# vdBerg93/cl-rrt

Measured on AMD Instinct MI355X. Metric: nodes expanded/sec (200-obstacle scene), higher is better.
Workload: dtype f64

## Files before the change

### cl-rrt_amd/csrc/clrrt_capi.hip

```cpp
#include <hip/hip_runtime.h>
#include <math.h>

#include <algorithm>
#include <climits>
#include <array>
#include <chrono>
#include <cmath>
#include <cstdio>
#include <cstdlib>
#include <cstring>
#include <deque>
#include <functional>
#include <optional>
#include <string>
#include <vector>

#include "../../include/clrrt.h"
#include "clrrt_dev.hpp"
#include "clrrt_internal.hpp"

static const int kWalkMaxOver = 2048, kWalkMaxChunks = 64;

using namespace clrrt;

// ... 60 lines not shown
  bool nnw_max_over_set = false;
  bool nnw_bud_tiles_set = false;
  int nnw_half_max = 4096;
  int nnw_hscale = 50;
  int nnw_lpt = 0;
  int nnw_index = 5;
  int nnw_lds_floor = 0;
  int nnw_waves = -1;
  int nnw_double = 1;
  WalkBufs nnw{};
  WalkBufs nnw_alt{};
  struct { int64_t n = -1; double ox, oy, x0, y0, x1, y1; float delta; } nnw_built;
  CompactBufs cmp{};
  int roll_persistent = 1;
  int nn_debug = 0;
  int roll_blocks = 0;
  int n_cu = 256;
  int* roll_q = nullptr;
  int* roll_best = nullptr;
  int roll_priority = 1;
  int roll_coop = 1;
  int roll_spread = 1;
  int roll_lanes = 0;
  int nn_exact_fused = 1;
  int exact_min_width = 8;
  int exact_fixup = 1;
  int exact_fix_cap = 0;
  int* fix_n = nullptr;
  int* fix_ids = nullptr;
  int* fix_adj = nullptr;
  NnRec* fix_xrec = nullptr;
  int* fix_xi = nullptr;
  int* fix_xcand = nullptr;
  float* fix_xkey = nullptr;
  int* fix_xn = nullptr;
  std::vector<int> h_fix_cand;
  std::vector<RollRes> h_fix_spec;
  Job* fix_jobs = nullptr;
  RollRes* fix_res = nullptr;
  std::vector<int> h_fix;
  std::vector<clrrt_sample> h_fix_smp;
  std::vector<Job> h_fix_jobs;
  std::vector<int> h_fix_owner;
  std::vector<RollRes> h_fix_res;
  std::vector<SampleOut> h_fix_so;
  int64_t ex_stats[10] = {0, 0, 0, 0, 0, 0, 0, 0, 0, 0};
  int* roll_perm = nullptr;
  int* roll_pflag = nullptr;
  GoalRec* goal_recs = nullptr;
  int* bp_path = nullptr;
  clrrt_node* path_nodes = nullptr;
  double* path_rows = nullptr;
  int path_cap = 0;
  int64_t path_rows_cap = 0;
  int path_n = 0;
  int64_t path_nrows = 0;
  int* ri_int = nullptr;
  int64_t* ri_off = nullptr;
  float* ri_cost = nullptr;
  double* ri_terms = nullptr;
  double reg_x0 = 0, reg_y0 = 0, reg_x1 = 0, reg_y1 = 0;
  int nn_pipeline = 1;
  hipStream_t side = nullptr;
  int cu_split = 0;
  hipStream_t roll_st = nullptr;
  hipEvent_t ev_rs0 = nullptr, ev_rs1 = nullptr;
  hipEvent_t ev_tree = nullptr, ev_walk = nullptr, ev_commit = nullptr;
  clrrt_sample* d_samples2 = nullptr;
  clrrt_sample* h_samples2 = nullptr;
  int* cand2 = nullptr;
  float* ckey2 = nullptr;
  int* ncand2 = nullptr;
  int* ctie2 = nullptr;
  int nn_lag = 0;
  clrrt_sample* d_samples3 = nullptr;
  clrrt_sample* h_samples3 = nullptr;
  int* cand3 = nullptr;
  float* ckey3 = nullptr;
  int* ncand3 = nullptr;
  int* ctie3 = nullptr;
  WalkBufs nnw3{};
  hipStream_t side2 = nullptr;
  hipStream_t mst = nullptr;
  int nn_split_delta = 0;
  int nn_delta_early = 1;
  int nn_lane_order = 1;
  int* nn_order = nullptr;
  float* wseed[3] = {nullptr, nullptr, nullptr};
  hipEvent_t ev_wm[3] = {nullptr, nullptr, nullptr};
  float* nn_seed2 = nullptr;
  float* d1pk[3] = {nullptr, nullptr, nullptr};
  int* d1pi[3] = {nullptr, nullptr, nullptr};
  hipEvent_t ev_d1[3] = {nullptr, nullptr, nullptr};
  hipEvent_t ev_s[3] = {nullptr, nullptr, nullptr};
  hipEvent_t ev_lagw[3] = {nullptr, nullptr, nullptr};
  int stream_prio = 1;
  int walk_cu_reserve = 0;
  hipEvent_t ev_lag[3] = {nullptr, nullptr, nullptr};
  int stream_prio_applied = 0;
  bool side_prio_set = false;
  std::vector<clrrt_sample> pf_next, pf_samples;
  int pf_state = 0;
  struct {
    int T = 0;
    bool active = false;
    int R = 0;
    int T_alloc = 0, n_steps_alloc = 0;
    int64_t vcap = 0;
    RollRes* res = nullptr;
    RollRes* res_gb = nullptr;
    int* cand = nullptr;
    int* ncand = nullptr;
    clrrt_sample* samp = nullptr;
    int* best = nullptr;
    int* dlist[2] = {nullptr, nullptr};
    int cur_dl = 0, nd = 0;
    int nd_eval = -1;
    int* gv = nullptr;
    uint8_t* pend = nullptr;
    void* sel_tmp = nullptr;
    size_t sel_bytes = 0;
    int* d_cnt = nullptr;
    void* carry[2] = {nullptr, nullptr};
    int cur_c = 0, ncarry = 0, carry_cap = 0;
    int64_t round = 0;
    int slot = 0;
    int64_t deferred_total = 0;
  } def;
  struct {
    int rank = 0, world = 1;
    void* dev_local = nullptr;
    int cap_local = 0;
    clrrt_exchange_fn fn = nullptr;
    void* user = nullptr;
    double max_ms = 0;
    int64_t nd_global = 0;
    int64_t rows_stop = 0;
    int last_nb = 0;
    clrrt_node* xbuf = nullptr;
    uint32_t* xkey = nullptr;
    void* xtmp = nullptr;
    size_t xtmp_bytes = 0;
    int64_t xcap = 0;
    unsigned long long* d_goal = nullptr;
    bool poison_seen = false;
    bool fn_failed = false;
  } sh;
  int fail_at_round = 0;
  int fail_after_exchange = 0;
  bool debug_sync = false;
  unsigned long long* dbg_host = nullptr;
  bool iter_log = false;
  std::vector<int64_t> round_sizes;
  std::vector<clrrt_iteration> iters;
  std::vector<SampleOut> iter_tmp;
  clrrt_sample* h_samples = nullptr;
  int64_t* h_totals = nullptr;
  int* h_int = nullptr;
  int64_t last_eval_rows = 0;
  int64_t last_goal_nodes = 0;
  clrrt_counters counters{};
  int64_t nn_bf_keys = 0, nn_samples = 0;
  int64_t nn_super_bounds = 0;
  bool timing = false;
  static constexpr int kKtClasses = 6;
  double kt_ms[kKtClasses] = {};
  int64_t kt_n[kKtClasses] = {};
  std::vector<hipEvent_t> ev_pool;
  std::vector<std::pair<int, std::pair<hipEvent_t, hipEvent_t>>> ev_pending;
};

static void pf_reset(clrrt_ctx* c);
static int flush_replays(clrrt_ctx* c);
static int append_nodes(clrrt_ctx* c, const clrrt_node* dev_nodes, int n);
static int watchdog_check(clrrt_ctx* c);
static void defer_roll_args(clrrt_ctx* c, RollArgs& a, bool capped);
static int commit_round(clrrt_ctx* c, int nn, double elapsed_ms, int* n_app);
// ... 160 lines not shown
  s[31] = 3;
  s[32] = 0;
  s[33] = 0;
  g->pos = 0;
  for (int i = 0; i < 310; i++) clrrt_rng_next(g);
}

int32_t clrrt_rng_next(clrrt_rng* g) {
  int32_t* s = g->r;
  int f = s[31], r = s[32];
  uint32_t v = (uint32_t)s[f] + (uint32_t)s[r];
  s[f] = (int32_t)v;
  int32_t out = (int32_t)(v >> 1);
  f = f + 1 == 31 ? 0 : f + 1;
  r = r + 1 == 31 ? 0 : r + 1;
  s[31] = f;
  s[32] = r;
  return out;
}

int clrrt_draw_samples(const clrrt_params* p, clrrt_rng* rng, int32_t n, clrrt_sample* out) {
  if (!p || !rng || (n > 0 && !out)) return CLRRT_EINVAL;
  const double* g = p->goal;
  const double RM = 2147483647.0;
  double dGoal = sqrt(g[0] * g[0] + g[1] * g[1]);
  double hd = atan2(g[1], g[0]);
  double latMin = -7, latMax = 7;
  float fl = (float)(RM / (dGoal + 10));
  float fw = (float)(RM / (latMax - latMin));
  double ch, sh, cq, sq;
  ::sincos(hd, &sh, &ch);
  ::sincos(hd + M_PI / 2, &sq, &cq);
  for (int j = 0; j < n; j++) {
    double rLong = (float)clrrt_rng_next(rng) / fl;
    double rLat = latMin + (float)clrrt_rng_next(rng) / fw;
    out[j].x = rLong * ch + rLat * cq;
    out[j].y = rLong * sh + rLat * sq;
    double r = (double)clrrt_rng_next(rng) / (double)(2147483647 / 1);
    out[j].explore = r <= ((0 * 0.3) + (1 * 0.7));
    out[j].pad = 0;
  }
  return CLRRT_OK;
}

const char* clrrt_last_error(const clrrt_ctx* c) { return c ? c->err.c_str() : "null context"; }

static void free_all(clrrt_ctx* c) {
  if (c->side) hipStreamSynchronize(c->side);
  void* ptrs[] = {c->tree, c->nn, c->arena, c->obs, c->d_samples, c->pk, c->pi, c->cand, c->ckey, c->ncand,
                  c->ctie, c->sort_scratch, c->res_spec, c->regnodes, c->res_gb, c->gbnodes, c->so, c->first_conflict,
                  c->out_nodes, c->jobs, c->slots, c->rep_buf, c->totals, c->work_ctr, c->grid_buf,
                  c->nn_seed, c->d_bbox, c->roll_q, c->roll_best, c->roll_perm, c->roll_pflag,
                  c->goal_recs, c->bp_path, c->path_nodes, c->path_rows, c->ri_int, c->ri_off, c->ri_cost,
                  c->ri_terms, c->nnw.keys, c->nnw.keys2, c->nnw.vals, c->nnw.vals2, c->nnw.tmp, c->nnw.P, c->nnw.Q,
                  c->nnw.CE, c->nnw.ID, c->nnw.tiles, c->nnw.supers, c->nnw.sorder, c->nnw.HEAD, c->nnw.ovf_n, c->nnw.ovf, c->nnw.pk, c->nnw.pi, c->nnw_alt.keys, c->nnw_alt.keys2, c->nnw_alt.vals, c->nnw_alt.vals2, c->nnw_alt.tmp, c->nnw_alt.P, c->nnw_alt.Q, c->nnw_alt.CE, c->nnw_alt.ID, c->nnw_alt.tiles, c->nnw_alt.supers, c->nnw_alt.sorder, c->nnw_alt.HEAD, c->nnw_alt.ovf_n, c->nnw_alt.ovf, c->nnw_alt.pk, c->nnw_alt.pi, c->nnw.skeys, c->nnw.sids, c->nnw_alt.skeys, c->nnw_alt.sids, c->cmp.packed, c->cmp.scanned,
                  c->cmp.tmp, c->d_samples2, c->cand2, c->ckey2, c->ncand2, c->ctie2, c->d_samples3, c->cand3, c->ckey3,
                  c->ncand3, c->ctie3, c->nnw3.keys, c->nnw3.keys2, c->nnw3.vals, c->nnw3.vals2, c->nnw3.tmp, c->nnw3.P,
                  c->nnw3.Q, c->nnw3.CE, c->nnw3.ID, c->nnw3.tiles, c->nnw3.supers, c->nnw3.sorder, c->nnw3.HEAD,
                  c->nnw3.ovf_n, c->nnw3.ovf, c->nnw3.pk, c->nnw3.pi, c->nnw3.skeys, c->nnw3.sids,
                  c->nnw.trun, c->nnw_alt.trun, c->nnw3.trun, c->nnw.wctr, c->nnw_alt.wctr, c->nnw3.wctr};
  for (void* p : ptrs)
    if (p) hipFree(p);
  void* sptrs[] = {c->sh.xbuf, c->sh.xkey, c->sh.xtmp, c->sh.d_goal, c->fix_n, c->fix_ids, c->fix_jobs, c->fix_res, c->fix_adj,
                   c->fix_xrec, c->fix_xi, c->fix_xcand, c->fix_xkey, c->fix_xn};
  for (void* p : sptrs)
    if (p) hipFree(p);
  void* dptrs[] = {c->def.res, c->def.res_gb, c->def.cand, c->def.ncand, c->def.samp, c->def.best, c->def.dlist[0],
                   c->def.dlist[1], c->def.gv, c->def.pend, c->def.sel_tmp, c->def.d_cnt, c->def.carry[0],
                   c->def.carry[1]};
  for (void* p : dptrs)
    if (p) hipFree(p);
  if (c->h_samples) hipHostFree(c->h_samples);
  if (c->h_samples2) hipHostFree(c->h_samples2);
  if (c->h_samples3) hipHostFree(c->h_samples3);
  if (c->side2) hipStreamSynchronize(c->side2);
  if (c->side2) hipStreamDestroy(c->side2);
  for (auto e : c->ev_lag)
    if (e) hipEventDestroy(e);
  for (auto e : c->ev_lagw)
    if (e) hipEventDestroy(e);
  if (c->mst) hipStreamSynchronize(c->mst);
  if (c->mst) hipStreamDestroy(c->mst);
  for (int q = 0; q < 3; q++) {
    if (c->ev_d1[q]) hipEventDestroy(c->ev_d1[q]);
    if (c->ev_s[q]) hipEventDestroy(c->ev_s[q]);
    if (c->d1pk[q]) hipFree(c->d1pk[q]);
    if (c->wseed[q]) hipFree(c->wseed[q]);
    if (q == 0 && c->nn_order) hipFree(c->nn_order);
    if (c->ev_wm[q]) hipEventDestroy(c->ev_wm[q]);
    if (c->d1pi[q]) hipFree(c->d1pi[q]);
  }
  if (c->nn_seed2) hipFree(c->nn_seed2);
  if (c->side) hipStreamSynchronize(c->side);
  if (c->ev_tree) hipEventDestroy(c->ev_tree);
  if (c->ev_walk) hipEventDestroy(c->ev_walk);
  if (c->ev_commit) hipEventDestroy(c->ev_commit);
  if (c->side) hipStreamDestroy(c->side);
  if (c->roll_st) hipStreamDestroy(c->roll_st);
  if (c->ev_rs0) hipEventDestroy(c->ev_rs0);
  if (c->ev_rs1) hipEventDestroy(c->ev_rs1);
  if (c->h_totals) hipHostFree(c->h_totals);
  if (c->h_int) hipHostFree(c->h_int);
  if (c->h_bbox) hipHostFree(c->h_bbox);
  if (c->dbg_host) hipHostFree(c->dbg_host);
  for (auto& pe : c->ev_pending) { hipEventDestroy(pe.second.first); hipEventDestroy(pe.second.second); }
  for (auto e : c->ev_pool) hipEventDestroy(e);
  if (c->own_stream && c->stream) hipStreamDestroy(c->stream);
}

int clrrt_create(const clrrt_params* p, const clrrt_capacity* cap, int device, clrrt_ctx** out) {
  if (!p || !out) return CLRRT_EINVAL;
  *out = nullptr;
  int ndev = 0;
  if (hipGetDeviceCount(&ndev) != hipSuccess || ndev <= 0) return CLRRT_EHIP;
  if (device < 0 || device >= ndev) return CLRRT_EINVAL;
  clrrt_ctx* c = new clrrt_ctx();
  c->device = device;
  c->params = *p;
  c->debug_sync = getenv("CLRRT_DEBUG_SYNC") != nullptr;
  clrrt_capacity dc;
  dc.max_nodes = 1 << 20;
  dc.max_rows = 1 << 24;
  dc.max_batch = 4096;
  dc.max_obstacles = 4096;
  c->cap = cap ? *cap : dc;
  if (c->cap.max_nodes < 2 || c->cap.max_rows < 2 || c->cap.max_batch < 1 || c->cap.max_obstacles < 0) {
    delete c;
    return CLRRT_EINVAL;
  }
  derive(c->params, c->dp, 0);
  int rc = CLRRT_OK;
  auto chk = [&](hipError_t e) {
    if (e != hipSuccess && rc == CLRRT_OK) { rc = CLRRT_EHIP; c->err = hipGetErrorString(e); }
  };
  chk(hipSetDevice(device));
  chk(hipStreamCreateWithFlags(&c->stream, hipStreamNonBlocking));
  c->own_stream = true;
  const int64_t B = c->cap.max_batch;
  chk(dalloc(&c->tree, c->cap.max_nodes));
  chk(dalloc(&c->nn, c->cap.max_nodes));
  chk(dalloc(&c->arena, (size_t)c->cap.max_rows * 10));
  chk(dalloc(&c->obs, std::max<int64_t>(1, c->cap.max_obstacles)));
  chk(dalloc(&c->d_samples, B));
  c->partial_cap = std::max<int64_t>(B * 16, 4096) * NN_K;
  chk(dalloc(&c->pk, c->partial_cap));
  chk(dalloc(&c->pi, c->partial_cap));
  chk(dalloc(&c->cand, B * CAND_K));
  chk(dalloc(&c->ckey, B * CAND_K));
  chk(dalloc(&c->ncand, B));
  chk(dalloc(&c->ctie, B));
  chk(dalloc(&c->d_samples2, B));
  chk(dalloc(&c->cand2, B * CAND_K));
  chk(dalloc(&c->ckey2, B * CAND_K));
  chk(dalloc(&c->ncand2, B));
  chk(dalloc(&c->ctie2, B));
  chk(hipStreamCreateWithFlags(&c->side, hipStreamNonBlocking));
  chk(hipEventCreateWithFlags(&c->ev_tree, hipEventDisableTiming));
  chk(hipEventCreateWithFlags(&c->ev_walk, hipEventDisableTiming));
  chk(hipEventCreateWithFlags(&c->ev_commit, hipEventDisableTiming));
  chk(dalloc(&c->res_spec, B * CAND_K));
  chk(dalloc(&c->regnodes, B));
  chk(dalloc(&c->res_gb, B * CAND_K));
  c->slot_rows = 0;
  chk(hipMalloc(&c->rep_buf, replay_bytes() * (size_t)2 * B));
  chk(dalloc(&c->gbnodes, B));
  chk(dalloc(&c->so, B));
  chk(dalloc(&c->first_conflict, 1));
  chk(dalloc(&c->out_nodes, 2 * B));
  chk(dalloc(&c->jobs, 2 * B));
  chk(dalloc(&c->totals, 8));
  chk(dalloc(&c->cmp.packed, B));
  chk(dalloc(&c->cmp.scanned, B));
  c->cmp.tmp_bytes = compact_scan_bytes((int)B);
  chk(hipMalloc(&c->cmp.tmp, std::max<size_t>(c->cmp.tmp_bytes, 256)));
  chk(dalloc(&c->nn_seed, B));
// ... 602 lines not shown

int clrrt_work_counters(clrrt_ctx* c, int64_t out[3]) {
  if (!c || !out) return CLRRT_EINVAL;
  HIPC(c, hipSetDevice(c->device));
  unsigned long long h[4];
  HIPC(c, hipMemcpyAsync(h, c->work_ctr, sizeof(h), hipMemcpyDeviceToHost, c->stream));
  HIPC(c, hipStreamSynchronize(c->stream));
  for (int i = 0; i < 3; i++) out[i] = (int64_t)h[i];
  return CLRRT_OK;
}

int clrrt_search_work(clrrt_ctx* c, int64_t out[4]) {
  if (!c || !out) return CLRRT_EINVAL;
  HIPC(c, hipSetDevice(c->device));
  HIPC(c, hipStreamSynchronize(c->stream));
  if (c->side) HIPC(c, hipStreamSynchronize(c->side));
  unsigned long long h[19];
  HIPC(c, hipMemcpy(h, c->work_ctr + 8, sizeof(h), hipMemcpyDeviceToHost));
  out[0] = c->nn_bf_keys;
  out[1] = c->nn_samples;
  out[2] = (int64_t)h[11];
  out[3] = (int64_t)h[13];
  return CLRRT_OK;
}

int clrrt_search_work_ex(clrrt_ctx* c, int64_t out[8]) {
  if (!c || !out) return CLRRT_EINVAL;
  int64_t w[4];
  const int rc = clrrt_search_work(c, w);
  if (rc != CLRRT_OK) return rc;
  unsigned long long h[19];
  HIPC(c, hipMemcpy(h, c->work_ctr + 8, sizeof(h), hipMemcpyDeviceToHost));
  for (int i = 0; i < 4; i++) out[i] = w[i];
  out[4] = c->nn_super_bounds;
  out[5] = (int64_t)h[10];
  out[6] = (int64_t)h[12];
  out[7] = 0;
  return CLRRT_OK;
}

int clrrt_nn_stats(clrrt_ctx* c, int64_t out[19]) {
  if (!c || !out) return CLRRT_EINVAL;
  HIPC(c, hipSetDevice(c->device));
  HIPC(c, hipStreamSynchronize(c->stream));
  unsigned long long h[19];
  HIPC(c, hipMemcpy(h, c->work_ctr + 8, sizeof(h), hipMemcpyDeviceToHost));
  for (int i = 0; i < 19; i++) out[i] = (int64_t)h[i];
  out[4] &= 0xffffffff;
  return CLRRT_OK;
}

int clrrt_set_option(clrrt_ctx* c, const char* key, int64_t value) {
  if (!c || !key) return CLRRT_EINVAL;
  const std::string k(key);
  if (k == "roll_persistent") c->roll_persistent = value != 0;
  else if (k == "nn_walk_min" && value >= 0) c->nnw_min_nodes = value;
  else if (k == "nn_walk_stateless") c->nnw_stateless = value != 0;
  else if (k == "nn_walk_budget_tiles" && value >= 0 && value < INT_MAX) {
    c->nnw_bud_tiles = (int)value;
    c->nnw_bud_tiles_set = true;
  }
  else if (k == "nn_walk_budget_keys" && value >= 0 && value < INT_MAX) c->nnw_bud_ex = (int)value;
  else if (k == "nn_walk_half_max" && value >= 0 && value < INT_MAX) c->nnw_half_max = (int)value;
  else if (k == "nn_walk_hscale" && value >= 1 && value <= 10000) {
    c->nnw_hscale = (int)value;
    c->nnw_built.n = -1;
    c->nnw.sorted_n = c->nnw_alt.sorted_n = c->nnw3.sorted_n = -1;
  }
  else if (k == "nn_walk_lpt") c->nnw_lpt = value != 0;
  else if (k == "nn_walk_index" && value >= 0 && value <= 5) {
    c->nnw_index = (int)value;
    c->nnw_built.n = -1;
    c->nnw.sorted_n = c->nnw_alt.sorted_n = c->nnw3.sorted_n = -1;
  }
  else if (k == "nn_walk_lds_floor" && value >= 0 && value <= 65536) c->nnw_lds_floor = (int)value;
  else if (k == "nn_walk_waves" && value >= -1 && value <= 1 << 20) c->nnw_waves = (int)value;
  else if (k == "nn_walk_chunks" && value >= 1 && value <= kWalkMaxChunks) c->nnw_chunks = (int)value;
  else if (k == "nn_walk_max_over" && value >= 1 && value <= kWalkMaxOver) {
    c->nnw_max_over = (int)value;
    c->nnw_max_over_set = true;
  }
  else if (k == "nn_walk_double") c->nnw_double = value != 0;
  else if (k == "nn_lag" && (value == 0 || value == 1 || value == 2)) c->nn_lag = (int)value;
  else if (k == "nn_split_delta") c->nn_split_delta = value != 0 ? 1 : 0;
  else if (k == "nn_delta_early") c->nn_delta_early = value != 0 ? 1 : 0;
  else if (k == "nn_lane_order") c->nn_lane_order = value != 0 ? 1 : 0;
  else if (k == "nn_debug" && value >= 0) c->nn_debug = (int)value;
  else if (k == "fail_at_round" && value >= 0 && value < INT_MAX) c->fail_at_round = (int)value;
  else if (k == "fail_after_exchange" && value >= 0 && value < INT_MAX) c->fail_after_exchange = (int)value;
  else if (k == "roll_blocks" && value >= 0 && value < (1 << 20)) c->roll_blocks = (int)value;
  else if (k == "nn_pipeline") c->nn_pipeline = value != 0;
  else if (k == "roll_priority") c->roll_priority = value != 0;
  else if (k == "roll_coop") c->roll_coop = value != 0;
  else if (k == "roll_spread") c->roll_spread = value != 0;
  else if (k == "roll_lanes") c->roll_lanes = (int)std::max<int64_t>(0, std::min<int64_t>(64, value));
  else if (k == "nn_exact_fused") c->nn_exact_fused = value != 0;
  else if (k == "rows_deferred") {
    int rc = flush_replays(c);
    if (rc != CLRRT_OK) return rc;
    c->rows_deferred = value != 0;
  }
  else if (k == "exact_min_width" && value >= 1 && value <= 1 << 20) c->exact_min_width = (int)value;
  else if (k == "exact_fixup") c->exact_fixup = value != 0;
  else if (k == "exact_fixup_cap" && value >= 0 && value < INT_MAX) c->exact_fix_cap = (int)value;
  else if (k == "defer_steps" && value >= 0 && value <= 1 << 20) {
    if (value > 0 && value < 8) return fail(c, CLRRT_EINVAL, "defer_steps must be 0 or >= 8");
    c->def.T = (int)value;
  }
  else if (k == "cu_split" && value >= 0 && value <= 7) {
    HIPC(c, hipStreamSynchronize(c->side));
    if (c->roll_st) HIPC(c, hipStreamSynchronize(c->roll_st));
    HIPC(c, hipStreamDestroy(c->side));
    c->side = nullptr;
    if (c->roll_st) HIPC(c, hipStreamDestroy(c->roll_st));
    c->roll_st = nullptr;
    c->cu_split = (int)value;
    c->stream_prio_applied = 0;
    if (value == 0) {
      HIPC(c, hipStreamCreateWithFlags(&c->side, hipStreamNonBlocking));
    } else {
      const int nw = (c->n_cu + 31) / 32;
      std::vector<uint32_t> mr(nw, 0u), ms(nw, 0u);
      for (int i = 0; i < c->n_cu; i++) ((i % 8) < value ? mr : ms)[i / 32] |= 1u << (i % 32);
      HIPC(c, hipExtStreamCreateWithCUMask(&c->roll_st, (uint32_t)nw, mr.data()));
      HIPC(c, hipExtStreamCreateWithCUMask(&c->side, (uint32_t)nw, ms.data()));
      if (!c->ev_rs0) HIPC(c, hipEventCreateWithFlags(&c->ev_rs0, hipEventDisableTiming));
      if (!c->ev_rs1) HIPC(c, hipEventCreateWithFlags(&c->ev_rs1, hipEventDisableTiming));
    }
  }
  else if (k == "stream_prio") c->stream_prio = value != 0;
  else if (k == "walk_cu_reserve" && value >= 0 && value <= 7) c->walk_cu_reserve = (int)value;
  else if (k == "side_priority") {
    int lo = 0, hi = 0;
    HIPC(c, hipDeviceGetStreamPriorityRange(&lo, &hi));
    HIPC(c, hipStreamSynchronize(c->side));
    HIPC(c, hipStreamDestroy(c->side));
    const int pr = value > 0 ? hi : value < 0 ? lo : 0;
    HIPC(c, hipStreamCreateWithPriority(&c->side, hipStreamNonBlocking, pr));
    c->side_prio_set = true;
    c->stream_prio_applied = 0;
    if (value < 0 && c->own_stream) {
      HIPC(c, hipStreamSynchronize(c->stream));
      HIPC(c, hipStreamDestroy(c->stream));
      HIPC(c, hipStreamCreateWithPriority(&c->stream, hipStreamNonBlocking, hi));
    }
  }
  else return fail(c, CLRRT_EINVAL, "unknown option or value: " + k);
  return CLRRT_OK;
}

int clrrt_enable_timing(clrrt_ctx* c, int32_t on) {
  if (!c) return CLRRT_EINVAL;
  drain_timers(c);
  c->timing = on != 0;
  for (int i = 0; i < clrrt_ctx::kKtClasses; i++) { c->kt_ms[i] = 0; c->kt_n[i] = 0; }
  return CLRRT_OK;
}

int clrrt_kernel_time(clrrt_ctx* c, int32_t which, double* ms, int64_t* launches) {
  if (!c || which < 0 || which >= clrrt_ctx::kKtClasses) return CLRRT_EINVAL;
  drain_timers(c);
  if (ms) *ms = c->kt_ms[which];
  if (launches) *launches = c->kt_n[which];
  return CLRRT_OK;
}

}
// ... 996 lines not shown
  c->sh.poison_seen = c->sh.fn_failed = false;
}

static int commit_round(clrrt_ctx* c, int nn, double elapsed_ms, int* n_app) {
  auto& h = c->sh;
  *n_app = 0;
  if (h.world <= 1) {
    *n_app = nn;
    const int rc = append_nodes(c, c->out_nodes, nn);
    if (rc == CLRRT_OK) c->round_sizes.push_back(c->n_nodes);
    return rc;
  }
  if (nn > h.cap_local) return fail(c, CLRRT_ECAPACITY, "the round's records exceed the exchange buffer");
  std::optional<KTimer> kt;
  kt.emplace(c, 5);
  if (nn > 0)
    HIPC(c, hipMemcpyAsync(h.dev_local, c->out_nodes, sizeof(clrrt_node) * nn, hipMemcpyDeviceToDevice, c->stream));
  clrrt_exchange_io io;
  memset(&io, 0, sizeof(io));
  io.n_local = nn;
  io.elapsed_ms = elapsed_ms;
  const int64_t nd_loc = c->def.active ? c->def.nd : 0;
  const bool rows_full =
      c->n_rows + nn + 2 * ((int64_t)h.last_nb + nd_loc) * (c->dp.n_steps_max + 1) > c->cap.max_rows;
  io.aux_local = nd_loc + (rows_full ? (1ll << 32) : 0);
  for (int q = 0; q < 4; q++) io.bbox_local[q] = nn > 0 ? c->h_bbox[q] : (q < 2 ? HUGE_VAL : -HUGE_VAL);
  io.stream = (void*)c->stream;
  io.max_elapsed_ms = elapsed_ms;
  io.aux_sum = io.aux_local;
  if (h.fn(h.user, &io) != 0 || io.n_all < 0 || (io.n_all > 0 && !io.dev_all)) {
    h.fn_failed = true;
    return fail(c, CLRRT_EHIP, "the exchange of the round's records failed");
  }
  kt.reset();
  const int64_t aux_sum = io.aux_sum;
  if (aux_sum >> 48) {
    h.poison_seen = true;
    return fail(c, CLRRT_EHIP, "sharded expansion: " + std::to_string(aux_sum >> 48) + " rank(s) failed this round");
  }
  if (c->fail_after_exchange > 0 && --c->fail_after_exchange == 0)
    return fail(c, CLRRT_ECAPACITY, "injected failure (option fail_after_exchange)");
  h.max_ms = io.max_elapsed_ms;
  h.nd_global = aux_sum & 0xffffffffll;
  h.rows_stop = (aux_sum >> 32) & 0xffff;
  const int32_t n_all = io.n_all;
  void* all = io.dev_all;
  if (n_all > 0) {
    if (n_all > h.xcap) {
      HIPC(c, hipStreamSynchronize(c->stream));
      for (void* p : {(void*)h.xbuf, (void*)h.xkey, h.xtmp})
        if (p) HIPC(c, hipFree(p));
      h.xbuf = nullptr; h.xkey = nullptr; h.xtmp = nullptr;
      const int64_t cap = std::max<int64_t>(2 * (int64_t)n_all, 4096);
      HIPC(c, dalloc(&h.xbuf, cap));
      HIPC(c, dalloc(&h.xkey, 4 * cap));
      h.xtmp_bytes = xorder_sort_bytes((int)cap);
      HIPC(c, hipMalloc(&h.xtmp, std::max<size_t>(h.xtmp_bytes, 256)));
      h.xcap = cap;
    }
    HIPC(c, launch_xorder(c->stream, (const clrrt_node*)all, n_all, c->def.active, h.xkey, h.xtmp, h.xtmp_bytes,
                          h.xbuf, h.d_goal));
    int rc = append_nodes(c, h.xbuf, n_all);
    if (rc != CLRRT_OK) return rc;
    bbox_add(c, io.bbox_all[0], io.bbox_all[1], io.bbox_all[2], io.bbox_all[3]);
  }
  *n_app = n_all;
  c->round_sizes.push_back(c->n_nodes);
  return CLRRT_OK;
}

struct LagSlot {
  clrrt_sample* d = nullptr;
  clrrt_sample* h = nullptr;
  int* cand = nullptr;
  float* ckey = nullptr;
  int* ncand = nullptr;
  int* ctie = nullptr;
  hipEvent_t ev = nullptr;
  hipEvent_t evw = nullptr;
  int n = 0;
  int64_t g = 0;
  int64_t tree_n = 0;
  int stream = 0;
  float* d1pk = nullptr;
  int* d1pi = nullptr;
  int d1_chunks = 0;
  int64_t d1_count = 0;
  hipEvent_t evd1 = nullptr;
  hipEvent_t evs = nullptr;
  float* wseed = nullptr;
  hipEvent_t evm = nullptr;
};

static int lag_alloc(clrrt_ctx* c) {
  if (c->side2) return CLRRT_OK;
  const int64_t B = c->cap.max_batch;
  HIPC(c, dalloc(&c->d_samples3, B));
  HIPC(c, dalloc(&c->cand3, B * CAND_K));
  HIPC(c, dalloc(&c->ckey3, B * CAND_K));
  HIPC(c, dalloc(&c->ncand3, B));
  HIPC(c, dalloc(&c->ctie3, B));
  HIPC(c, hipHostMalloc((void**)&c->h_samples3, sizeof(clrrt_sample) * B, hipHostMallocDefault));
  for (auto& e : c->ev_lag) HIPC(c, hipEventCreateWithFlags(&e, hipEventDisableTiming));
  for (auto& e : c->ev_lagw) HIPC(c, hipEventCreateWithFlags(&e, hipEventDisableTiming));
  if (c->cu_split > 0) {
    const int nw = (c->n_cu + 31) / 32;
    std::vector<uint32_t> ms(nw, 0u);
    for (int i = 0; i < c->n_cu; i++)
      if ((i % 8) >= c->cu_split) ms[i / 32] |= 1u << (i % 32);
    HIPC(c, hipExtStreamCreateWithCUMask(&c->side2, (uint32_t)nw, ms.data()));
  } else {
    HIPC(c, hipStreamCreateWithFlags(&c->side2, hipStreamNonBlocking));
  }
  HIPC(c, hipStreamCreateWithFlags(&c->mst, hipStreamNonBlocking));
  HIPC(c, dalloc(&c->nn_seed2, B));
  for (int q = 0; q < 3; q++) {
    HIPC(c, dalloc(&c->d1pk[q], c->partial_cap));
    HIPC(c, dalloc(&c->wseed[q], B));
    if (q == 0) HIPC(c, dalloc(&c->nn_order, B));
    HIPC(c, hipEventCreateWithFlags(&c->ev_wm[q], hipEventDisableTiming));
    HIPC(c, dalloc(&c->d1pi[q], c->partial_cap));
    HIPC(c, hipEventCreateWithFlags(&c->ev_d1[q], hipEventDisableTiming));
    HIPC(c, hipEventCreateWithFlags(&c->ev_s[q], hipEventDisableTiming));
  }
  return CLRRT_OK;
}

static int apply_stream_prio(clrrt_ctx* c) {
  const int want = (c->stream_prio ? 1 : 2) + 4 * c->walk_cu_reserve;
  if (c->stream_prio_applied == want || c->cu_split > 0) return CLRRT_OK;
  int lo = 0, hi = 0;
  HIPC(c, hipDeviceGetStreamPriorityRange(&lo, &hi));
  const int p_hi = c->stream_prio ? hi : 0, p_lo = c->stream_prio ? lo : 0;
  HIPC(c, hipDeviceSynchronize());
  auto remake = [&](hipStream_t& st, int pr) -> int {
    if (st) HIPC(c, hipStreamDestroy(st));
    HIPC(c, hipStreamCreateWithPriority(&st, hipStreamNonBlocking, pr));
    return CLRRT_OK;
  };
  int rc;
  if (c->walk_cu_reserve > 0) {
    const int nw = (c->n_cu + 31) / 32;
    std::vector<uint32_t> ms(nw, 0u);
    for (int i = 0; i < c->n_cu; i++)
      if ((i % 8) >= c->walk_cu_reserve) ms[i / 32] |= 1u << (i % 32);
    for (hipStream_t* st : {&c->side, &c->side2}) {
      if (*st) HIPC(c, hipStreamDestroy(*st));
      HIPC(c, hipExtStreamCreateWithCUMask(st, (uint32_t)nw, ms.data()));
    }
    if ((rc = remake(c->mst, p_hi)) != CLRRT_OK) return rc;
  } else if ((!c->side_prio_set && (rc = remake(c->side, p_lo)) != CLRRT_OK) ||
             (rc = remake(c->side2, p_lo)) != CLRRT_OK || (rc = remake(c->mst, p_hi)) != CLRRT_OK) {
    return rc;
  }
  if (c->own_stream && (rc = remake(c->stream, p_hi)) != CLRRT_OK) return rc;
  c->stream_prio_applied = want;
  return CLRRT_OK;
}

static int expand_lag2(clrrt_ctx* c, clrrt_rng* rng, int64_t n_iters, double budget_ms, int32_t batch,
                       clrrt_stats* out) {
  int rc = lag_alloc(c);
  if (rc == CLRRT_OK) rc = apply_stream_prio(c);
  if (rc == CLRRT_OK) rc = defer_begin(c, true);
  if (rc != CLRRT_OK) return rc;
  clrrt_stats st{};
  const auto t0 = std::chrono::steady_clock::now();
  clrrt_rng work = *rng, committed = *rng;
  std::deque<clrrt_sample> pending;
  const int cur = batch;
  const bool sharded = c->sh.world > 1;
  c->sh.max_ms = 0;
  c->sh.nd_global = 0;
  c->sh.rows_stop = 0;
  shard_expansion_begin(c);
  if (sharded && (rc = shard_goal_reset(c)) != CLRRT_OK) return rc;
  const int64_t nodes_before = c->n_nodes;
  hipStream_t sides[2] = {c->side, c->side2};
  WalkBufs* W[3] = {&c->nnw, &c->nnw_alt, &c->nnw3};
  int64_t built_n[3] = {-1, -1, -1};
  double built_f[3][7] = {};
  LagSlot A, B;
  A.d = c->d_samples2; A.h = c->h_samples2; A.cand = c->cand2; A.ckey = c->ckey2; A.ncand = c->ncand2;
  A.ctie = c->ctie2; A.ev = c->ev_lag[0]; A.evw = c->ev_lagw[0];
  B.d = c->d_samples3; B.h = c->h_samples3; B.cand = c->cand3; B.ckey = c->ckey3; B.ncand = c->ncand3;
  B.ctie = c->ctie3; B.ev = c->ev_lag[1]; B.evw = c->ev_lagw[1];
  A.d1pk = c->d1pk[0]; A.d1pi = c->d1pi[0]; A.evd1 = c->ev_d1[0]; A.evs = c->ev_s[0];
  B.d1pk = c->d1pk[1]; B.d1pi = c->d1pi[1]; B.evd1 = c->ev_d1[1]; B.evs = c->ev_s[1];
  A.wseed = c->wseed[0]; A.evm = c->ev_wm[0];
  B.wseed = c->wseed[1]; B.evm = c->ev_wm[1];
  float* cur_wseed = c->wseed[2];
  hipEvent_t cur_evm = c->ev_wm[2];
  const bool early = c->nn_delta_early != 0;
  hipEvent_t cur_ev = c->ev_lag[2];
  hipEvent_t cur_evw = c->ev_lagw[2];
  float* cur_d1pk = c->d1pk[2];
  int* cur_d1pi = c->d1pi[2];
  hipEvent_t cur_evd1 = c->ev_d1[2], cur_evs = c->ev_s[2];
  const bool split_delta = c->nn_split_delta != 0;
  struct RoleGuard {
    std::function<void()> f;
    ~RoleGuard() { f(); }
  } role_guard{[&]() {
    c->d_samples2 = A.d; c->h_samples2 = A.h; c->cand2 = A.cand; c->ckey2 = A.ckey; c->ncand2 = A.ncand; c->ctie2 = A.ctie;
    c->d_samples3 = B.d; c->h_samples3 = B.h; c->cand3 = B.cand; c->ckey3 = B.ckey; c->ncand3 = B.ncand; c->ctie3 = B.ctie;
    c->ev_lag[0] = A.ev; c->ev_lag[1] = B.ev; c->ev_lag[2] = cur_ev;
    c->ev_lagw[0] = A.evw; c->ev_lagw[1] = B.evw; c->ev_lagw[2] = cur_evw;
    c->nnw_built.n = -1;
    c->nnw.sorted_n = -1;
    c->nnw_alt.sorted_n = -1;
    c->nnw3.sorted_n = -1;
  }};
  bool have_cur = false;
  int cur_stream = 0;
  double last_round_ms = 0;
  auto frame_of = [](const NnSetup& su, double* f) {
    f[0] = su.fr.ox; f[1] = su.fr.oy; f[2] = su.fr.delta; f[3] = su.x0; f[4] = su.y0; f[5] = su.x1; f[6] = su.y1;
  };
  auto build = [&](int k, const NnSetup& su) -> int {
    double f[7];
    frame_of(su, f);
    if (built_n[k] == c->n_nodes && std::equal(f, f + 7, built_f[k])) return CLRRT_OK;
    int r2 = ensure_walk_set(c, *W[k]);
    if (r2 != CLRRT_OK) return r2;
    const WalkBufs* prev = nullptr;
    for (int q = 1; q <= 2 && !prev; q++) {
      const WalkBufs* w = W[(k + 3 - q) % 3];
      if (w->P && w->sorted_n > 0) prev = w;
    }
    KTimer kt(c, 0, c->stream);
    HIPC(c, launch_nn_walk_build(c->stream, c->nn, (int)c->n_nodes, su.fr, su.x0, su.y0, su.x1, su.y1, *W[k], prev));
    built_n[k] = c->n_nodes;
    std::copy(f, f + 7, built_f[k]);
    return CLRRT_OK;
  };
  auto walk = [&](LagSlot& sl, int n, int k, const NnSetup& su, int si) -> int {
    hipStream_t s = sides[si];
    int r2 = ensure_walk_set(c, *W[k]);
    if (r2 != CLRRT_OK) return r2;
    c->nn_bf_keys += (int64_t)n * c->n_nodes;
    c->nn_samples += n;
    HIPC(c, hipStreamWaitEvent(s, c->ev_tree, 0));
    HIPC(c, hipMemcpyAsync(sl.d, sl.h, sizeof(clrrt_sample) * n, hipMemcpyHostToDevice, s));
    HIPC(c, hipEventRecord(sl.evs, s));
    sl.d1_count = 0;
    sl.d1_chunks = 0;
    c->nn_super_bounds += (int64_t)n * walk_super_count(c->n_nodes);
    {
      KTimer kt(c, 0, s), kt3(c, 3, s);
      W[k]->seed_out = early ? sl.wseed : nullptr;
      W[k]->ev_main = early ? sl.evm : nullptr;
      const hipError_t ew = launch_nn_walk_search(s, sl.d, n, c->nn, (int)c->n_nodes, c->dp, su.fr, su.x0, su.y0, su.x1,
                                                  su.y1, *W[k], sl.cand, sl.ckey, sl.ncand, sl.ctie, c->work_ctr + 18,
                                                  c->nnw_stateless);
      W[k]->seed_out = nullptr;
      W[k]->ev_main = nullptr;
      HIPC(c, ew);
    }
    HIPC(c, hipEventRecord(sl.evw, s));
    sl.n = n;
    sl.tree_n = c->n_nodes;
    sl.stream = si;
    return CLRRT_OK;
  };
  auto draw_to = [&](int64_t want) {
    while ((int64_t)pending.size() < want) {
      clrrt_sample smp;
      clrrt_draw_samples(&c->params, &work, 1, &smp);
      pending.push_back(smp);
    }
  };
  for (int64_t k = 0; rc == CLRRT_OK; k++) {
    const auto tr0 = std::chrono::steady_clock::now();
    if (n_iters > 0 && st.iterations >= n_iters) break;
    const double ms0 = std::chrono::duration<double, std::milli>(tr0 - t0).count();
    if (n_iters == 0 && !((sharded ? c->sh.max_ms : ms0) < budget_ms)) break;
    const int64_t left = n_iters > 0 ? n_iters - st.iterations : INT64_MAX;
    const int64_t gb = std::min<int64_t>(cur, left);
    int64_t f0 = 0;
    int nb = (int)gb;
    if (sharded) shard_slice(c, gb, &f0, &nb);
    c->sh.last_nb = nb;
    const int64_t nc = gb + (sharded ? c->sh.nd_global : (int64_t)c->def.nd);
    if (c->n_nodes + 2 * nc > c->cap.max_nodes ||
        (sharded ? c->sh.rows_stop > 0 : c->n_rows + 2 * nc * (c->dp.n_steps_max + 1) > c->cap.max_rows)) {
      if (n_iters > 0) { rc = fail(c, CLRRT_ECAPACITY, "tree capacity exhausted"); break; }
      st.capacity_stop = 1;
      break;
    }
    const int wk = (int)(k % 3);
    const NnSetup su = nn_setup(c);
    const bool serve = c->n_nodes >= c->nnw_min_nodes && su.region_ok;
    int64_t gA = 0, gB = 0, fA = 0, fB = 0;
    int nA = 0, nB = 0;
    if (serve) {
      const bool more = n_iters > 0 || ms0 + 2.0 * last_round_ms < budget_ms;
      if (A.n == 0 && (n_iters > 0 || ms0 + last_round_ms < budget_ms)) gA = std::max<int64_t>(0, std::min<int64_t>(cur, left - gb));
      const int64_t gA_eff = A.n > 0 ? A.g : gA;
      if (more && gA_eff > 0) gB = std::max<int64_t>(0, std::min<int64_t>(cur, left - gb - gA_eff));
      nA = (int)gA;
      nB = (int)gB;
      if (sharded) {
        shard_slice(c, gA, &fA, &nA);
        shard_slice(c, gB, &fB, &nB);
      }
    }
    const int64_t gA_all = A.n > 0 ? A.g : gA;
    draw_to(gb + gA_all + gB);
    if (have_cur) {
      KTimer kt(c, 4);
      HIPC(c, hipStreamWaitEvent(c->stream, cur_ev, 0));
    } else {
      for (int j = 0; j < nb; j++) c->h_samples[j] = pending[f0 + j];
      HIPC(c, hipMemcpyAsync(c->d_samples, c->h_samples, sizeof(clrrt_sample) * nb, hipMemcpyHostToDevice, c->stream));
      if (serve) {
        HIPC(c, hipStreamSynchronize(c->side));
        HIPC(c, hipStreamSynchronize(c->side2));
        HIPC(c, hipStreamSynchronize(c->mst));
        if ((rc = build(wk, su)) != CLRRT_OK) break;
        c->nn_bf_keys += (int64_t)nb * c->n_nodes;
        c->nn_samples += nb;
        c->nn_super_bounds += (int64_t)nb * walk_super_count(c->n_nodes);
        KTimer kt(c, 0), kt3(c, 3);
        HIPC(c, launch_nn_walk_search(c->stream, c->d_samples, nb, c->nn, (int)c->n_nodes, c->dp, su.fr, su.x0, su.y0,
                                      su.x1, su.y1, *W[wk], c->cand, c->ckey, c->ncand, c->ctie, c->work_ctr + 18,
                                      c->nnw_stateless));
      } else if ((rc = run_nn(c, nb, nullptr)) != CLRRT_OK) {
        break;
      }
    }
    if (serve && (nA > 0 || nB > 0) && (rc = build(wk, su)) != CLRRT_OK) break;
    auto ahead = [&]() -> int {
      if (nA > 0) {
        for (int j = 0; j < nA; j++) A.h[j] = pending[gb + fA + j];
        const int r2 = walk(A, nA, wk, su, cur_stream);
        if (r2 != CLRRT_OK) return r2;
        A.g = gA;
      }
      if (nB > 0) {
        for (int j = 0; j < nB; j++) B.h[j] = pending[gb + gA_all + fB + j];
        const int r2 = walk(B, nB, wk, su, nA > 0 ? A.stream : 1 - A.stream);
        if (r2 != CLRRT_OK) return r2;
        B.g = gB;
      }
      return CLRRT_OK;
    };
    int L = nb, nn = 0, n_app = 0;
    if ((rc = eval_samples(c, nb, false, &L, true, (nA > 0 || nB > 0) ? std::function<int()>(ahead) : nullptr,
                           nullptr)) != CLRRT_OK)
      break;
    if ((rc = compact_and_copy(c, L, &nn, true)) != CLRRT_OK) break;
    const double ms_commit = std::chrono::duration<double, std::milli>(std::chrono::steady_clock::now() - t0).count();
    if ((rc = commit_round(c, nn, ms_commit, &n_app)) != CLRRT_OK) break;
    if ((A.n > 0 || (split_delta && B.n > 0)))
      HIPC(c, hipEventRecord(c->ev_commit, c->stream));
    if (A.n > 0 && split_delta) {
      hipStream_t s = c->mst;
      HIPC(c, hipStreamWaitEvent(s, c->ev_commit, 0));
      HIPC(c, hipStreamWaitEvent(s, early ? A.evm : A.evw, 0));
      const int64_t first2 = A.tree_n + A.d1_count, cnt2 = c->n_nodes - first2;
      int nch2 = 0;
      if (cnt2 > 0) {
        KTimer kt(c, 0, s);
        c->nn_bf_keys += (int64_t)A.n * cnt2;
        const NnSetup su2 = nn_setup(c);
        const int max_chunks = (int)std::max<int64_t>(1, c->partial_cap / ((int64_t)A.n * NN_K));
        HIPC(c, launch_nn_delta_partial(s, A.d, A.n, c->nn, (int)first2, (int)cnt2, c->dp, su2.fr, c->pk, c->pi,
                                        max_chunks, A.ckey, A.ncand, early ? A.wseed : c->nn_seed, early,
                                        c->nn_lane_order ? c->nn_order : nullptr, &nch2));
      }
      if (early) HIPC(c, hipStreamWaitEvent(s, A.evw, 0));
      if (A.d1_count > 0) HIPC(c, hipStreamWaitEvent(s, A.evd1, 0));
      {
        KTimer kt(c, 0, s);
        if (A.d1_count > 0)
          HIPC(c, launch_nn_delta_merge(s, A.n, A.d1_chunks, c->dp, A.d1pk, A.d1pi, (int)A.tree_n, A.cand, A.ckey,
                                        A.ncand, A.ctie));
        HIPC(c, launch_nn_delta_merge(s, A.n, nch2, c->dp, c->pk, c->pi, (int)first2, A.cand, A.ckey, A.ncand, A.ctie));
      }
      HIPC(c, hipEventRecord(A.ev, s));
    } else if (A.n > 0 && early) {
      hipStream_t s = c->mst;
      HIPC(c, hipStreamWaitEvent(s, c->ev_commit, 0));
      HIPC(c, hipStreamWaitEvent(s, A.evm, 0));
      const int64_t first = A.tree_n, cnt = c->n_nodes - A.tree_n;
      int nch = 0;
      if (cnt > 0) {
        KTimer kt(c, 0, s);
        c->nn_bf_keys += (int64_t)A.n * cnt;
        const NnSetup su2 = nn_setup(c);
        const int max_chunks = (int)std::max<int64_t>(1, c->partial_cap / ((int64_t)A.n * NN_K));
        HIPC(c, launch_nn_delta_partial(s, A.d, A.n, c->nn, (int)first, (int)cnt, c->dp, su2.fr, c->pk, c->pi,
                                        max_chunks, nullptr, nullptr, A.wseed, true,
                                        c->nn_lane_order ? c->nn_order : nullptr, &nch));
      }
      HIPC(c, hipStreamWaitEvent(s, A.evw, 0));
      {
        KTimer kt(c, 0, s);
        HIPC(c, launch_nn_delta_merge(s, A.n, nch, c->dp, c->pk, c->pi, (int)first, A.cand, A.ckey, A.ncand, A.ctie));
      }
      HIPC(c, hipEventRecord(A.ev, s));
    } else if (A.n > 0) {
      hipStream_t s = c->mst;
      HIPC(c, hipStreamWaitEvent(s, c->ev_commit, 0));
      HIPC(c, hipStreamWaitEvent(s, A.evw, 0));
      const int64_t first = A.tree_n, cnt = c->n_nodes - A.tree_n;
      if (cnt > 0) {
        KTimer kt(c, 0, s);
        c->nn_bf_keys += (int64_t)A.n * cnt;
        const NnSetup su2 = nn_setup(c);
        const int max_chunks = (int)std::max<int64_t>(1, c->partial_cap / ((int64_t)A.n * NN_K));
        HIPC(c, launch_nn_delta(s, A.d, A.n, c->nn, (int)first, (int)cnt, c->dp, su2.fr, c->pk, c->pi, max_chunks,
                                A.cand, A.ckey, A.ncand, A.ctie, c->nn_seed));
      }
      HIPC(c, hipEventRecord(A.ev, s));
    }
    if (split_delta && B.n > 0) {
      hipStream_t s2 = c->mst;
      HIPC(c, hipStreamWaitEvent(s2, c->ev_commit, 0));
      HIPC(c, hipStreamWaitEvent(s2, B.evs, 0));
      HIPC(c, hipStreamWaitEvent(s2, early ? B.evm : B.evw, 0));
      const int64_t cnt1 = c->n_nodes - B.tree_n;
      B.d1_count = cnt1;
      B.d1_chunks = 0;
      if (cnt1 > 0) {
        KTimer kt(c, 0, s2);
        c->nn_bf_keys += (int64_t)B.n * cnt1;
        const NnSetup su1 = nn_setup(c);
        const int max_chunks = (int)std::max<int64_t>(1, c->partial_cap / ((int64_t)B.n * NN_K));
        HIPC(c, launch_nn_delta_partial(s2, B.d, B.n, c->nn, (int)B.tree_n, (int)cnt1, c->dp, su1.fr, B.d1pk, B.d1pi,
                                        max_chunks, B.ckey, B.ncand, early ? B.wseed : c->nn_seed2, early,
                                        c->nn_lane_order ? c->nn_order : nullptr, &B.d1_chunks));
      }
      HIPC(c, hipEventRecord(B.evd1, s2));
    }
    {
      const NnSetup sn = nn_setup(c);
      if (B.n > 0 && c->n_nodes >= c->nnw_min_nodes && sn.region_ok && (rc = build((int)((k + 1) % 3), sn)) != CLRRT_OK)
        break;
    }
    for (int64_t j = 0; j < gb; j++) {
      pending.pop_front();
      for (int q = 0; q < 3; q++) clrrt_rng_next(&committed);
    }
    st.iterations += gb;
    st.goal_nodes_added += c->last_goal_nodes;
    st.speculated += gb;
    st.rounds++;
    {
      LagSlot old;
      old.d = c->d_samples; old.h = c->h_samples; old.cand = c->cand; old.ckey = c->ckey; old.ncand = c->ncand;
      old.ctie = c->ctie; old.ev = cur_ev; old.evw = cur_evw; old.stream = cur_stream;
      old.d1pk = cur_d1pk; old.d1pi = cur_d1pi; old.evd1 = cur_evd1; old.evs = cur_evs;
      old.wseed = cur_wseed; old.evm = cur_evm;
      have_cur = A.n > 0;
      c->d_samples = A.d; c->h_samples = A.h; c->cand = A.cand; c->ckey = A.ckey; c->ncand = A.ncand; c->ctie = A.ctie;
      cur_ev = A.ev;
      cur_evw = A.evw;
      cur_stream = A.stream;
      cur_d1pk = A.d1pk; cur_d1pi = A.d1pi; cur_evd1 = A.evd1; cur_evs = A.evs;
      cur_wseed = A.wseed; cur_evm = A.evm;
      A = B;
      B = old;
      B.n = 0;
      B.stream = 1 - A.stream;
    }
    last_round_ms = std::chrono::duration<double, std::milli>(std::chrono::steady_clock::now() - tr0).count();
  }
  if (rc == CLRRT_OK) rc = defer_drain(c, &st.goal_nodes_added);
  st.deferred = c->def.deferred_total;
  if (rc == CLRRT_OK) rc = flush_replays(c);
  if (rc == CLRRT_OK && sharded) rc = shard_goal_count(c, &st.goal_nodes_added);
  rc = shard_expansion_end(c, rc);
  c->def.active = false;
  for (hipStream_t s : {c->side, c->side2, c->mst, c->stream}) {
    const hipError_t e = hipStreamSynchronize(s);
    if (e != hipSuccess && rc == CLRRT_OK) rc = fail(c, CLRRT_EHIP, std::string("hipStreamSynchronize: ") + hipGetErrorString(e));
  }
  st.nodes_added = c->n_nodes - nodes_before;
  st.elapsed_ms = std::chrono::duration<double, std::milli>(std::chrono::steady_clock::now() - t0).count();
  *rng = committed;
  if (out) *out = st;
  return rc;
}

int clrrt_expand(clrrt_ctx* c, clrrt_rng* rng, int64_t n_iters, double budget_ms, int32_t mode, int32_t batch,
                 clrrt_stats* out) {
  if (!c || !rng || n_iters < 0 || (mode != CLRRT_MODE_EXACT && mode != CLRRT_MODE_BATCH)) return CLRRT_EINVAL;
  pf_reset(c);
  if (n_iters == 0 && !(budget_ms > 0)) return CLRRT_EINVAL;
  if (c->n_nodes <= 0) return fail(c, CLRRT_ESTATE, "tree not initialised");
  c->round_sizes.clear();
  const bool sharded = c->sh.world > 1;
  if (sharded && mode != CLRRT_MODE_BATCH) return fail(c, CLRRT_EINVAL, "sharded expansion runs BATCH rounds only");
  HIPC(c, hipSetDevice(c->device));
  const int64_t bmax = (int64_t)c->cap.max_batch * c->sh.world;
  batch = (int32_t)std::max<int64_t>(1, std::min<int64_t>(batch > 0 ? batch : bmax, bmax));
  if (sharded && batch < c->sh.world) return fail(c, CLRRT_EINVAL, "fewer samples per round than ranks");
  const int lag = c->nn_lag ? c->nn_lag
                  : (n_iters == 0 ? budget_ms >= 1000.0 : n_iters >= 64 * (int64_t)batch) ? 2 : 1;
  if (mode == CLRRT_MODE_BATCH && c->nn_pipeline && lag == 2) return expand_lag2(c, rng, n_iters, budget_ms, batch, out);
  clrrt_stats st{};
  auto t0 = std::chrono::steady_clock::now();
  clrrt_rng work = *rng;
  clrrt_rng committed = *rng;
  std::deque<clrrt_sample> pending;
  const bool exact = mode == CLRRT_MODE_EXACT;
  int cur = exact ? std::min(batch, std::max(16, c->exact_min_width)) : batch;
  int64_t nodes_before = c->n_nodes;
  int rc = defer_begin(c, !exact);
  c->sh.max_ms = 0;
  c->sh.nd_global = 0;
  c->sh.rows_stop = 0;
  shard_expansion_begin(c);
  if (rc == CLRRT_OK && sharded) rc = shard_goal_reset(c);
  bool have_next = false;
  double last_round_ms = 0;
  auto draw_to = [&](int64_t want) {
    while ((int64_t)pending.size() < want) {
      clrrt_sample smp;
      clrrt_draw_samples(&c->params, &work, 1, &smp);
      pending.push_back(smp);
    }
  };
  for (; rc == CLRRT_OK;) {
    const auto tr0 = std::chrono::steady_clock::now();
    if (n_iters > 0 && st.iterations >= n_iters) break;
    if (n_iters == 0) {
      double ms = std::chrono::duration<double, std::milli>(std::chrono::steady_clock::now() - t0).count();
      if (!((sharded ? c->sh.max_ms : ms) < budget_ms)) break;
    }
    int64_t gb = cur;
    if (n_iters > 0) gb = std::min<int64_t>(gb, n_iters - st.iterations);
    int64_t f0 = 0;
    int nb = (int)gb;
    if (sharded) shard_slice(c, gb, &f0, &nb);
    c->sh.last_nb = nb;
    const int64_t nc = gb + (sharded ? c->sh.nd_global : (int64_t)c->def.nd);
    if (c->n_nodes + 2 * nc > c->cap.max_nodes ||
        (sharded ? c->sh.rows_stop > 0 : c->n_rows + 2 * nc * (c->dp.n_steps_max + 1) > c->cap.max_rows)) {
      if (n_iters > 0) { rc = fail(c, CLRRT_ECAPACITY, "tree capacity exhausted"); break; }
      st.capacity_stop = 1;
      break;
// ... 357 lines not shown
```

### cl-rrt_amd/csrc/clrrt_internal.hpp

```cpp
#pragma once
#include <hip/hip_runtime.h>
#include <stdint.h>

#include "../../include/clrrt.h"
#include "clrrt_dev.hpp"
#include "clrrt_stdsort.hpp"

namespace clrrt {

#define CLRRT_ROLL_PENDING (-2)

struct RollRes {
  double st[10];
  double costE, costS;
  double bx, by;
  double fx, fy;
  double vback;
  int32_t outcome;
  int32_t nrows;
  int32_t refN;
  int32_t pad;
};

struct WorkCtr {
// ... 87 lines not shown
  const float* __restrict__ ckey;
  const int* __restrict__ ncand;
  const RollRes* __restrict__ res;
  const RollRes* __restrict__ res_gb;
  clrrt_node* regnodes;
  clrrt_node* gbnodes;
  SampleOut* so;
  int B;
  const int* view;
  int nd, sbase;
  int* gv;
  uint8_t* pend;
  int* new_pend;
};

struct NnFrame {
  double ox, oy;
  float delta;
  int debug;
};
struct WalkTile {
  float pcx, pcy, pr;
  float rcx, rcy, rr;
  float thx, thy, thh;
  float apx, apy, aph;
  float cemin;
  float aopt;
  int32_t nonfinite;
  float eroot;
};
static_assert(sizeof(WalkTile) == 64, "WalkTile layout");
struct WalkBufs {
  uint32_t *keys, *keys2;
  int *vals, *vals2;
  int* sorder;
  void* tmp;
  size_t tmp_bytes;
  float4 *P, *Q;
  float* CE;
  int* ID;
  int* HEAD;
  int2* trun;
  WalkTile *tiles, *supers;
  int bud_tiles, bud_ex, max_over, nch;
  int half_max = 4096;
  int lds_floor = 0;
  int waves = 0;
  int waves_min_batch = 0;
  int index_kind = 0;
  int hscale_pct = 100;
  int* wctr = nullptr;
  int lpt = 0;
  float* seed_out = nullptr;
  hipEvent_t ev_main = nullptr;
  int* ovf_n;
  int4* ovf;
  float* pk;
  int* pi;
  uint64_t* skeys;
  int* sids;
  int64_t sorted_n;
  double sorted_x0, sorted_y0, sorted_scale;
  int sorted_kind;
  int64_t cap_nodes;
  int cap_batch;
};
size_t walk_sort_bytes(int n);
int64_t walk_tile_count(int64_t n);
int64_t walk_super_count(int64_t n);
hipError_t launch_nn_walk(hipStream_t st, const clrrt_sample* S, int B, const NnRec* nodes, int N, const DevParams& p,
                          const NnFrame& fr, double x0, double y0, double x1, double y1, WalkBufs& w, int* cand,
                          float* ckey, int* ncand, int* ctie, unsigned long long* stats, bool stateless);
hipError_t launch_nn_walk_build(hipStream_t st, const NnRec* nodes, int N, const NnFrame& fr, double x0, double y0,
                                double x1, double y1, WalkBufs& w, const WalkBufs* prev = nullptr);
hipError_t launch_nn_walk_search(hipStream_t st, const clrrt_sample* S, int B, const NnRec* nodes, int N,
                                 const DevParams& p, const NnFrame& fr, double x0, double y0, double x1, double y1,
                                 WalkBufs& w, int* cand, float* ckey, int* ncand, int* ctie, unsigned long long* stats,
                                 bool stateless);
hipError_t launch_walk_audit(hipStream_t st, const clrrt_sample* S, int B, const NnRec* nodes, int N, const DevParams& p,
                             const NnFrame& fr, const WalkBufs& w, int* out);
hipError_t launch_nn_delta(hipStream_t st, const clrrt_sample* S, int B, const NnRec* nodes, int first, int count,
                           const DevParams& p, const NnFrame& fr, float* pk, int* pi, int max_chunks, int* cand,
                           float* ckey, int* ncand, int* ctie, float* seed);
hipError_t launch_nn_delta_partial(hipStream_t st, const clrrt_sample* S, int B, const NnRec* nodes, int first,
                                   int count, const DevParams& p, const NnFrame& fr, float* pk, int* pi, int max_chunks,
                                   const float* ckey, const int* ncand, float* gcap, bool seeded, int* order,
                                   int* nchunks_out);
hipError_t launch_nn_delta_merge(hipStream_t st, int B, int nchunks, const DevParams& p, const float* pk, const int* pi,
                                 int id0, int* cand, float* ckey, int* ncand, int* ctie);
hipError_t launch_nn(hipStream_t st, const clrrt_sample* S, int B, const NnRec* nodes, int N,
                     const DevParams& p, float* pk, int* pi, int* cand, float* ckey, int* ncand, int* ctie,
                     int max_chunks, KeyId* exact_scratch, float* seed, unsigned long long* stats, const NnFrame& fr);
hipError_t launch_nn_exact_only(hipStream_t st, const clrrt_sample* S, int B, const NnRec* nodes, int N,
                                const DevParams& p, const int* ctie, KeyId* scratch, int* cand, float* ckey,
                                int* ncand);
hipError_t launch_rollout(hipStream_t st, int src, const RollArgs& a);
hipError_t launch_nn_exact_small(hipStream_t st, const clrrt_sample* S, int B, const NnRec* nodes, int N,
                                 const DevParams& p, int* cand, float* ckey, int* ncand, int* ctie);
int nn_exact_small_max();
hipError_t launch_rollout_persistent(hipStream_t st, const RollArgs& a, int B, int* qnext, int* best, int blocks,
                                     bool prefilled = false);
struct FillInts {
  int* p[8];
  int n[8];
  int v[8];
  int nj = 0;
  void add(int* ptr, int count, int value) {
    if (ptr && count > 0) { p[nj] = ptr; n[nj] = count; v[nj] = value; nj++; }
  }
};
hipError_t launch_fill_ints(hipStream_t st, const FillInts& f);
size_t roll_order_scratch_bytes(int n);
size_t replay_bytes();
size_t carry_bytes();
hipError_t launch_replay_gather(hipStream_t st, const Job* jobs, const clrrt_node* recs, int n, const clrrt_node* tree,
                                const int* cand, const clrrt_sample* S, const RollRes* res, void* out);
hipError_t launch_select(hipStream_t st, const SelArgs& a);
hipError_t launch_copy_rows(hipStream_t st, const Job* jobs, const clrrt_node* recs, int n, const double* slots,
                            int slot_rows, int slot_jobs, double* arena);
#define FIX_MAX 4
hipError_t launch_nn_exact_x(hipStream_t st, const clrrt_sample* S, const NnRec* nodes, int N, const DevParams& p,
                             const clrrt_node* reg, const clrrt_node* gbn, const SampleOut* so, int n, NnRec* xrec,
                             const int* slist, const int* xcnt, int nlist, int xmax, int* cand, float* ckey,
                             int* ncand, int* ctie);
hipError_t launch_conflict_fix(hipStream_t st, const DevParams& p, int B, const clrrt_sample* S,
                               const clrrt_node* reg, const clrrt_node* gbn, const SampleOut* so, const int* ctie,
                               const int* ncand, const float* ckey, const RollRes* res, int* fix_n, int* fix_ids,
                               int* fix_adj);
hipError_t launch_conflict(hipStream_t st, const DevParams& p, int B, const clrrt_sample* S,
                           const clrrt_node* reg, const clrrt_node* gbn, const SampleOut* so, const int* ctie,
                           int* first);
struct CompactBufs {
  uint64_t* packed;
  uint64_t* scanned;
  void* tmp;
  size_t tmp_bytes;
};
size_t compact_scan_bytes(int n);
size_t defer_select_bytes(int n);
hipError_t launch_defer_select(hipStream_t st, const int* gv, const uint8_t* pend, int n, int* out, int* n_out,
                               void* tmp, size_t tmp_bytes);
hipError_t launch_compact(hipStream_t st, int L, const clrrt_sample* S, const int* cand, const clrrt_node* reg,
                          const clrrt_node* gbn, const SampleOut* so, int64_t row_base, int rank,
                          clrrt_node* out, Job* jobs, int64_t* totals, CompactBufs& cb, int tag_slot = 0,
                          int tag_R = 0, int tag_B = 1, bool totals_zeroed = false);
size_t xorder_sort_bytes(int n);
hipError_t launch_xorder(hipStream_t st, const clrrt_node* recs, int n, bool sort, uint32_t* keys, void* tmp,
                         size_t tmp_bytes, clrrt_node* out, unsigned long long* goal);
hipError_t launch_bbox(hipStream_t st, const clrrt_node* recs, const int64_t* n_dev, int n_host, double* out4);
hipError_t launch_append(hipStream_t st, const clrrt_node* in, int n, int64_t base, clrrt_node* tree, NnRec* nn);
hipError_t launch_selftest_math(hipStream_t st, int fn, const double* a, const double* b, int n, double* out);
hipError_t launch_obs_distance(hipStream_t st, const DevParams& p, const BakedObs* obs, const double* states, int n,
                               double* out);
hipError_t launch_selftest_units(hipStream_t st, int unit, const double* in, const BakedObs* obs, int n,
                                 const DevParams& p, const DevParams* cp, double* out);
struct GoalRec { int32_t id; float cost; };
hipError_t launch_goal_gather(hipStream_t st, const clrrt_node* tree, int64_t n, GoalRec* out, int* cnt);
hipError_t launch_backtrack(hipStream_t st, const clrrt_node* tree, int64_t n, int start, int cap, int* path,
                            int* len);
struct ReinitArgs {
  DevParams p;
  const BakedObs* obs;
  const clrrt_node* pn;
  int n;
  const double* prow;
  double car[10];
  clrrt_node* tree;
  NnRec* nn;
  double* arena;
  int* kidx;
// ... 15 lines not shown
```

### cl-rrt_amd/csrc/clrrt_kernels.hip

```cpp
#include <hip/hip_runtime.h>
#include <hipcub/hipcub.hpp>
#include <stddef.h>
#include <stdint.h>

#include "clrrt_dev.hpp"
#include "clrrt_internal.hpp"
#include "clrrt_stdsort.hpp"

namespace clrrt {

#define CAND_K 10
#define NN_K (CAND_K + 1)
static_assert(CAND_K == 10, "sortLimit");

__device__ __forceinline__ bool lex_less(float ka, int ia, float kb, int ib) {
  return (ka < kb) || (ka == kb && ia < ib);
}

__device__ __forceinline__ void topk_insert(float (&keys)[NN_K], int (&ids)[NN_K], float k, int i) {
#pragma unroll
  for (int j = 0; j < NN_K; j++) {
    bool sw = lex_less(k, i, keys[j], ids[j]);
    float tk = keys[j];
    int ti = ids[j];
// ... 203 lines not shown
                           const int* __restrict__ pi, int* __restrict__ cand, float* __restrict__ ckey,
                           int* __restrict__ ncand, int* __restrict__ ctie) {
  const int t = blockIdx.x * blockDim.x + threadIdx.x;
  if (t >= B) return;
  const int s = t;
  float keys[NN_K];
  int ids[NN_K];
#pragma unroll
  for (int j = 0; j < NN_K; j++) { keys[j] = __builtin_inff(); ids[j] = 0x7fffffff; }
  for (int c = 0; c < nchunks; c++) {
    size_t base = ((size_t)t * nchunks + c) * NN_K;
    for (int j = 0; j < NN_K; j++) {
      int id = pi[base + j];
      if (id == 0x7fffffff) break;
      float k = pk[base + j];
      if (lex_less(k, id, keys[NN_K - 1], ids[NN_K - 1])) topk_insert(keys, ids, k, id);
      else break;
    }
  }
  int n = 0, valid = 0;
#pragma unroll
  for (int j = 0; j < NN_K; j++) valid += ids[j] != 0x7fffffff;
  const int sel = min(limit, valid);
  int tie = 0;
#pragma unroll
  for (int j = 0; j < CAND_K; j++) {
    bool v = j < sel;
    cand[s * CAND_K + j] = v ? ids[j] : -1;
    ckey[s * CAND_K + j] = keys[j];
    n += v;
    tie |= (j < sel && j + 1 < valid && keys[j] == keys[j + 1]);
  }
  ncand[s] = n;
  ctie[s] = tie;
}

__global__ void k_nn_delta_seed(int B, int limit, const float* __restrict__ ckey, const int* __restrict__ ncand,
                                float* __restrict__ seed) {
  const int s = blockIdx.x * blockDim.x + threadIdx.x;
  if (s >= B) return;
  const float k = (limit > 0 && ncand[s] >= limit) ? ckey[s * CAND_K + limit - 1] : __builtin_inff();
  ((unsigned int*)seed)[s] = ord_enc32(k);
}

__global__ void k_nn_merge_delta(int B, int nchunks, int limit, const float* __restrict__ pk,
                                 const int* __restrict__ pi, int id0, int* __restrict__ cand,
                                 float* __restrict__ ckey, int* __restrict__ ncand, int* __restrict__ ctie) {
  const int s = blockIdx.x * blockDim.x + threadIdx.x;
  if (s >= B) return;
  float keys[NN_K];
  int ids[NN_K];
  const int n0 = ncand[s];
#pragma unroll
  for (int j = 0; j < NN_K; j++) {
    const bool v = j < CAND_K && j < n0;
    keys[j] = v ? ckey[s * CAND_K + (j < CAND_K ? j : 0)] : __builtin_inff();
    ids[j] = v ? cand[s * CAND_K + (j < CAND_K ? j : 0)] : 0x7fffffff;
  }
  for (int c = 0; c < nchunks; c++) {
    const size_t base = ((size_t)s * nchunks + c) * NN_K;
    for (int j = 0; j < NN_K; j++) {
      const int id = pi[base + j];
      if (id == 0x7fffffff) break;
      const float k = pk[base + j];
      if (lex_less(k, id + id0, keys[NN_K - 1], ids[NN_K - 1])) topk_insert(keys, ids, k, id + id0);
      else break;
    }
  }
  int n = 0, valid = 0;
#pragma unroll
  for (int j = 0; j < NN_K; j++) valid += ids[j] != 0x7fffffff;
  const int sel = min(limit, valid);
  int tie = 0;
#pragma unroll
  for (int j = 0; j < CAND_K; j++) {
    const bool v = j < sel;
    cand[s * CAND_K + j] = v ? ids[j] : -1;
    ckey[s * CAND_K + j] = keys[j];
    n += v;
    tie |= (j < sel && j + 1 < valid && keys[j] == keys[j + 1]);
  }
  ncand[s] = n;
  ctie[s] = tie;
}

__global__ void k_nn_exact(const clrrt_sample* __restrict__ S, int B, const NnRec* __restrict__ nodes, int N,
                           DevParams p, const int* __restrict__ ctie, KeyId* __restrict__ scratch,
                           int* __restrict__ cand, float* __restrict__ ckey, int* __restrict__ ncand) {
  const int s = blockIdx.x * blockDim.x + threadIdx.x;
  if (s >= B || !ctie[s]) return;
  const double sx = S[s].x, sy = S[s].y;
  const int ex = S[s].explore;
  KeyId* a = scratch + (size_t)s * N;
  for (int n = 0; n < N; n++) {
    const NnRec& rec = nodes[n];
    float k = dubins_key(sx, sy, rec.x, rec.y, rec.c, rec.s);
    if (!ex) k = rec.costE + k;
    a[n].id = n;
    a[n].key = k;
  }
  std_sort(a, N);
  int cnt = 0;
  for (int i = 0; i < N && cnt < p.sort_limit; i++) {
    const NnRec& rec = nodes[a[i].id];
    if (feasible_search(sx, sy, rec.bx, rec.by, rec.ca, rec.sa, rec.ang_par, p.feas_len)) {
      cand[s * CAND_K + cnt] = a[i].id;
      ckey[s * CAND_K + cnt] = a[i].key;
      cnt++;
    }
  }
  for (int j = cnt; j < CAND_K; j++) cand[s * CAND_K + j] = -1;
  ncand[s] = cnt;
}

__device__ __forceinline__ void wave_std_sort(KeyId* a, int n, int2* pairs, int need = INT_MAX) {
  const int lane = threadIdx.x & 63;
  if (n <= 1) return;
  int lim = n;
  struct Rg { int lo, hi, depth; };
  Rg stack[64];
  int sp = 0;
  int lo = 0, hi = n;
  int depth = 2 * ilog2(n);
  __shared__ int s_l[64], s_r[64];
  for (;;) {
    while (hi - lo > 16) {
      if (depth == 0) {
        if (lane == 0) heap_sort_(a + lo, hi - lo);
        __syncthreads();
        break;
      }
      --depth;
      if (lane == 0) {
        KeyId* first = a + lo;
        KeyId* last = a + hi;
        median_to_first_(first, first + 1, first + (last - first) / 2, last - 1);
      }
      __syncthreads();
      const float P = a[lo].key;
      const int f = lo + 1, l = hi;
      int lpos = f, rpos = l - 1;
      int nl = 0, hl = 0, nr = 0, hr = 0;
      int np = 0;
      int prevR = INT_MAX;
      int cut = -1;
      while (cut < 0) {
        if (nl == 0) {
          const int i = lpos + lane;
          const bool st = i < l && !(a[i].key < P);
          const uint64_t m = __ballot(st);
          if (st) s_l[__popcll(m & ((1ull << lane) - 1))] = i;
          nl = __popcll(m);
          hl = 0;
          lpos += 64;
        }
        if (nr == 0) {
          const int i = rpos - lane;
          const bool st = i >= f && !(P < a[i].key);
          const uint64_t m = __ballot(st);
          if (st) s_r[__popcll(m & ((1ull << lane) - 1))] = i;
          nr = __popcll(m);
          hr = 0;
          rpos -= 64;
        }
        __syncthreads();
        const bool lend = nl == 0 && lpos >= l, rend = nr == 0 && rpos < f;
// ... 2062 lines not shown
    e = launch_nn_brute(st, S, B, nodes, N, p, fr, pk, pi, cand, ckey, ncand, ctie, max_chunks, seed,
                        stats ? stats + 5 : nullptr);
    if (e != hipSuccess) return e;
  }
  if (exact_scratch) return launch_nn_exact_any(st, S, B, nodes, N, p, ctie, exact_scratch, cand, ckey, ncand);
  return hipSuccess;
}

hipError_t launch_nn_exact_small(hipStream_t st, const clrrt_sample* S, int B, const NnRec* nodes, int N,
                                 const DevParams& p, int* cand, float* ckey, int* ncand, int* ctie) {
  if (N > NN_EXACT_LDS_MAX || B <= 0) return hipErrorInvalidValue;
  const size_t lds = sizeof(KeyId) * (size_t)N + sizeof(int2) * (size_t)(N / 2 + 64);
  if (lds > 64 * 1024) {
    const hipError_t e = hipFuncSetAttribute((const void*)&k_nn_exact_fused, hipFuncAttributeMaxDynamicSharedMemorySize,
                                             (int)lds);
    if (e != hipSuccess) return e;
  }
  hipLaunchKernelGGL(k_nn_exact_fused, dim3(B), dim3(64), lds, st, S, B, nodes, N, p, cand, ckey, ncand, ctie);
  return hipGetLastError();
}

int nn_exact_small_max() { return NN_EXACT_LDS_MAX; }

__global__ void k_build_xrec(const clrrt_node* __restrict__ reg, const clrrt_node* __restrict__ gbn,
                             const SampleOut* __restrict__ so, int n, int64_t base, NnRec* __restrict__ xrec) {
  if (blockIdx.x != 0 || threadIdx.x != 0) return;
  int64_t pos = 0;
  for (int k = 0; k < n; k++) {
    if (so[k].k < 0) continue;
    xrec[pos] = nn_record(reg[k], base + pos);
    pos++;
    if (so[k].gb_ok) {
      xrec[pos] = nn_record(gbn[k], base + pos);
      pos++;
    }
  }
}

hipError_t launch_nn_exact_x(hipStream_t st, const clrrt_sample* S, const NnRec* nodes, int N, const DevParams& p,
                             const clrrt_node* reg, const clrrt_node* gbn, const SampleOut* so, int n, NnRec* xrec,
                             const int* slist, const int* xcnt, int nlist, int xmax, int* cand, float* ckey,
                             int* ncand, int* ctie) {
  if (nlist <= 0) return hipSuccess;
  const int Nl = N + xmax;
  if (Nl > NN_EXACT_LDS_MAX) return hipErrorInvalidValue;
  hipLaunchKernelGGL(k_build_xrec, dim3(1), dim3(64), 0, st, reg, gbn, so, n, (int64_t)N, xrec);
  LAUNCH_CHECK();
  const size_t lds = sizeof(KeyId) * (size_t)Nl + sizeof(int2) * (size_t)(Nl / 2 + 64);
  if (lds > 64 * 1024) {
    const hipError_t e = hipFuncSetAttribute((const void*)&k_nn_exact_fused, hipFuncAttributeMaxDynamicSharedMemorySize,
                                             (int)lds);
    if (e != hipSuccess) return e;
  }
  hipLaunchKernelGGL(k_nn_exact_fused, dim3(nlist), dim3(64), lds, st, S, nlist, nodes, N, p, cand, ckey, ncand, ctie,
                     (const NnRec*)xrec, xcnt, slist, Nl);
  return hipGetLastError();
}

hipError_t launch_nn_delta(hipStream_t st, const clrrt_sample* S, int B, const NnRec* nodes, int first, int count,
                           const DevParams& p, const NnFrame& fr, float* pk, int* pi, int max_chunks, int* cand,
                           float* ckey, int* ncand, int* ctie, float* seed) {
  if (count <= 0 || B <= 0) return hipSuccess;
  const int groups = (B + CLRRT_PATH_BLK - 1) / CLRRT_PATH_BLK;
  int nchunks = (count + 255) / 256;
  const int want = max(1, 2048 / max(1, groups));
  nchunks = max(1, min(nchunks, min(want, max_chunks)));
  int chunk = (count + nchunks - 1) / nchunks;
  chunk = (chunk + 255) & ~255;
  nchunks = (count + chunk - 1) / chunk;
  hipLaunchKernelGGL(k_nn_delta_seed, dim3((B + 63) / 64), dim3(64), 0, st, B, p.sort_limit, ckey, ncand, seed);
  LAUNCH_CHECK();
  hipLaunchKernelGGL(k_nn_partial, dim3(groups, nchunks), dim3(CLRRT_PATH_BLK), 0, st, S, B, nodes + first, count, chunk,
                     nchunks, p, fr, pk, pi, seed, nullptr, nullptr);
  LAUNCH_CHECK();
  hipLaunchKernelGGL(k_nn_merge_delta, dim3((B + 63) / 64), dim3(64), 0, st, B, nchunks, p.sort_limit, pk, pi,
                     first, cand, ckey, ncand, ctie);
  LAUNCH_CHECK();
  return hipSuccess;
}

hipError_t launch_nn_delta_partial(hipStream_t st, const clrrt_sample* S, int B, const NnRec* nodes, int first,
                                   int count, const DevParams& p, const NnFrame& fr, float* pk, int* pi, int max_chunks,
                                   const float* ckey, const int* ncand, float* gcap, bool seeded, int* order,
                                   int* nchunks_out) {
  *nchunks_out = 0;
  if (count <= 0 || B <= 0) return hipSuccess;
  const int* sord = nullptr;
  if (order) {
    hipLaunchKernelGGL(k_nn_order, dim3(1), dim3(1024), 0, st, S, B, order);
    LAUNCH_CHECK();
    sord = order;
  }
  const int groups = (B + CLRRT_PATH_BLK - 1) / CLRRT_PATH_BLK;
  int nchunks = (count + 255) / 256;
  const int want = max(1, 2048 / max(1, groups));
  nchunks = max(1, min(nchunks, min(want, max_chunks)));
  int chunk = (count + nchunks - 1) / nchunks;
  chunk = (chunk + 255) & ~255;
  nchunks = (count + chunk - 1) / chunk;
  if (!seeded) {
    hipLaunchKernelGGL(k_nn_delta_seed, dim3((B + 63) / 64), dim3(64), 0, st, B, ckey ? p.sort_limit : 0, ckey, ncand,
                       gcap);
    LAUNCH_CHECK();
  }
  hipLaunchKernelGGL(k_nn_partial, dim3(groups, nchunks), dim3(CLRRT_PATH_BLK), 0, st, S, B, nodes + first, count, chunk,
                     nchunks, p, fr, pk, pi, gcap, nullptr, sord);
  LAUNCH_CHECK();
  *nchunks_out = nchunks;
  return hipSuccess;
}
hipError_t launch_nn_delta_merge(hipStream_t st, int B, int nchunks, const DevParams& p, const float* pk, const int* pi,
                                 int id0, int* cand, float* ckey, int* ncand, int* ctie) {
  if (nchunks <= 0 || B <= 0) return hipSuccess;
  hipLaunchKernelGGL(k_nn_merge_delta, dim3((B + 63) / 64), dim3(64), 0, st, B, nchunks, p.sort_limit, pk, pi, id0, cand,
                     ckey, ncand, ctie);
  LAUNCH_CHECK();
  return hipSuccess;
}

hipError_t launch_nn_exact_only(hipStream_t st, const clrrt_sample* S, int B, const NnRec* nodes, int N,
                                const DevParams& p, const int* ctie, KeyId* scratch, int* cand, float* ckey,
                                int* ncand) {
  return launch_nn_exact_any(st, S, B, nodes, N, p, ctie, scratch, cand, ckey, ncand);
}

static hipError_t launch_nn_brute(hipStream_t st, const clrrt_sample* S, int B, const NnRec* nodes, int N,
                                  const DevParams& p, const NnFrame& fr, float* pk, int* pi, int* cand,
                                  float* ckey, int* ncand, int* ctie, int max_chunks, const float* seed,
                                  unsigned long long* tstat) {
  int threads = 256;
  int groups = (B + 255) / 256;
  int nchunks = (N + 255) / 256;
  int want = max(1, 2048 / max(1, groups));
  nchunks = max(1, min(nchunks, min(want, max_chunks)));

  int chunk = (N + nchunks - 1) / nchunks;
  chunk = (chunk + 255) & ~255;
  nchunks = (N + chunk - 1) / chunk;
  hipLaunchKernelGGL(k_nn_partial, dim3(groups, nchunks), dim3(threads), 0, st, S, B, nodes, N, chunk, nchunks,
                     p, fr, pk, pi, seed, tstat, nullptr);
  LAUNCH_CHECK();
  hipLaunchKernelGGL(k_nn_merge, dim3((B + 255) / 256), dim3(256), 0, st, B, nchunks, p.sort_limit, pk, pi,
                     cand, ckey, ncand, ctie);
  LAUNCH_CHECK();
  return hipSuccess;
}

static size_t roll_lds_bytes(const RollArgs& a) {
  size_t lds = 0;
  if (a.p.coll_mode == CLRRT_COLLISION_OBB) {
    lds = (size_t)a.p.n_obs * (6 * sizeof(float4) + sizeof(float));
    if (a.grid.gw > 0)
      lds += sizeof(uint32_t) * ((size_t)a.grid.gw * a.grid.gh + 1) +
             sizeof(uint16_t) * ((size_t)a.grid.nitems + a.grid.nmov);
  }
  return lds;
}

template <int SRC>
static hipError_t launch_roll_t(hipStream_t st, const RollArgs& a) {
  if (a.njobs <= 0) return hipSuccess;
  const size_t lds = roll_lds_bytes(a);
  const int64_t threads = (int64_t)a.njobs * (a.job_stride > 1 ? a.job_stride : 1);
  dim3 grid((unsigned)((threads + 255) / 256)), block(256);
  if (a.p.need_gap)
    hipLaunchKernelGGL((k_rollout<SRC, true>), grid, block, 0, st, a);
  else
  {
    if (lds > 64 * 1024) {
      hipError_t e = hipFuncSetAttribute((const void*)&k_rollout<SRC, false>,
                                         hipFuncAttributeMaxDynamicSharedMemorySize, (int)lds);
      if (e != hipSuccess) return e;
    }
    hipLaunchKernelGGL((k_rollout<SRC, false>), grid, block, lds, st, a);
  }
  LAUNCH_CHECK();
  return hipSuccess;
}

size_t roll_order_scratch_bytes(int n) {
  size_t bytes = 0;
  hipcub::DeviceScan::ExclusiveSum(nullptr, bytes, (const int*)nullptr, (int*)nullptr, n);
  return bytes;
}
static hipError_t roll_order(hipStream_t st, const RollArgs& a) {
  if (!a.perm || !a.pflag) return hipSuccess;
  int* ppos = a.pflag + a.njobs;
  void* tmp = (void*)(((uintptr_t)(a.pflag + 2 * (size_t)a.njobs) + 255) & ~(uintptr_t)255);
  size_t bytes = roll_order_scratch_bytes(a.njobs);
  hipError_t e = hipcub::DeviceScan::ExclusiveSum(tmp, bytes, a.pflag, ppos, a.njobs, st);
  if (e != hipSuccess) return e;
  hipLaunchKernelGGL(k_roll_order, dim3((a.njobs + 63) / 64), dim3(64), 0, st, a.pflag, ppos, a.njobs, a.perm);
  return hipGetLastError();
}

__global__ void __launch_bounds__(256) k_fill_ints(FillInts f) {
  const int stride = gridDim.x * blockDim.x;
  for (int q = 0; q < f.nj; q++)
// ... 272 lines not shown
```

### cl-rrt_amd/csrc/clrrt_nnwalk.hip

```cpp
#include <hip/hip_runtime.h>
#include <climits>
#include <hip/hip_fp16.h>
#include <hipcub/hipcub.hpp>
#include <rocprim/device/device_merge.hpp>
#include <algorithm>
#include <stdint.h>

#include "clrrt_dev.hpp"
#include "clrrt_internal.hpp"

namespace clrrt {

#define CAND_K 10
#define NN_K (CAND_K + 1)
#define WALK_TILE 32
#define WALK_SUPER 32
#define WALK_FMT_STATE 0
#define WALK_FMT_HALF 1
#define WALK_FMT_CODED 2
#ifndef WALK_STAGE1_QUEUE
#define WALK_STAGE1_QUEUE 0
#endif
#ifndef WALK_HALF_SUPER
#define WALK_HALF_SUPER 1
#endif
#define WALK_TQ 68
#ifndef WALK_SPLIT_SHARE
#define WALK_SPLIT_SHARE 1
#endif
#ifndef WALK_APBINS
#define WALK_APBINS 8
#endif
#ifndef WALK_SECTOR_BITS
#define WALK_SECTOR_BITS 3
#endif

#define LAUNCH_CHECK3()                          \
  do {                                           \
    hipError_t e_ = hipGetLastError();           \
    if (e_ != hipSuccess) return e_;             \
  } while (0)

__device__ __forceinline__ uint32_t w_spread(uint32_t v) {
  v &= 0xffff;
  v = (v | (v << 8)) & 0x00ff00ff;
  v = (v | (v << 4)) & 0x0f0f0f0f;
  v = (v | (v << 2)) & 0x33333333;
  v = (v | (v << 1)) & 0x55555555;
  return v;
}

__device__ __forceinline__ uint64_t w_spread3(uint32_t v) {
  uint64_t x = v & 0xffff;
  x = (x | (x << 16)) & 0x0000ff0000ffull;
  x = (x | (x << 8)) & 0x00f00f00f00full;
  x = (x | (x << 4)) & 0x0c30c30c30c3ull;
  x = (x | (x << 2)) & 0x249249249249ull;
  return x;
}

__global__ void k_walk_keys(const NnRec* __restrict__ nodes, int N, double x0, double y0, double scale,
                            uint64_t* __restrict__ keys, int* __restrict__ vals, int first = 0, int kind = 0,
                            double hrho = 4.77) {
  const int k0 = blockIdx.x * blockDim.x + threadIdx.x;
  if (k0 >= N - first) return;
  const int i = first + k0;
  keys += -first;
  vals += -first;
  const double x = nodes[i].x, y = nodes[i].y;
  const float apf = (float)nodes[i].ang_par;
  int bin = (int)floorf((apf + 3.14159265f) * (WALK_APBINS / 6.2831853f));
  bin = bin < 0 ? 0 : (bin >= WALK_APBINS ? WALK_APBINS - 1 : bin);
  if (kind >= 3) {
    const float ang = kind != 4 ? atan2f(-nodes[i].s, nodes[i].c) : apf;
    const double a = isfinite(ang) ? (double)ang - 6.283185307179586 * floor(((double)ang + M_PI) / 6.283185307179586)
                                   : 0.0;
    uint64_t m = 0xffffffffffffull;
    if (isfinite(x) && isfinite(y)) {
      const double fx = fmin(fmax((x - x0) * scale, 0.0), 65535.0);
      const double fy = fmin(fmax((y - y0) * scale, 0.0), 65535.0);
      const double fz = fmin(fmax((a + M_PI) * hrho * scale, 0.0), 65535.0);
      m = w_spread3((uint32_t)fx) | (w_spread3((uint32_t)fy) << 1) | (w_spread3((uint32_t)fz) << 2);
    }
    uint64_t low = __float_as_uint(nodes[i].costE) >> (16 + WALK_SECTOR_BITS);
    if (kind == 5) {
      const double bx = nodes[i].bx, by = nodes[i].by;
      uint32_t cx = 0, cy = 0;
      if (isfinite(bx) && isfinite(by)) {
        cx = (uint32_t)fmin(fmax((bx - x0) * scale, 0.0), 65535.0) >> 9;
        cy = (uint32_t)fmin(fmax((by - y0) * scale, 0.0), 65535.0) >> 10;
      }
      low = (w_spread(cx) | (w_spread(cy) << 1)) & 0x1fffu;
    }
    keys[i] = ((uint64_t)bin << (64 - WALK_SECTOR_BITS)) | (m << (16 - WALK_SECTOR_BITS)) | low;
    vals[i] = i;
    return;
  }
  if (kind != 0) {
    const float ang = kind == 1 ? atan2f(-nodes[i].s, nodes[i].c) : apf;
    const double a = isfinite(ang) ? (double)ang - 6.283185307179586 * floor(((double)ang + M_PI) / 6.283185307179586)
                                   : 0.0;
    uint64_t m = 0xffffffffffffull;
    if (isfinite(x) && isfinite(y)) {
      const double fx = fmin(fmax((x - x0) * scale, 0.0), 65535.0);
      const double fy = fmin(fmax((y - y0) * scale, 0.0), 65535.0);
      const double fz = fmin(fmax((a + M_PI) * hrho * scale, 0.0), 65535.0);
      m = w_spread3((uint32_t)fx) | (w_spread3((uint32_t)fy) << 1) | (w_spread3((uint32_t)fz) << 2);
    }
    keys[i] = (m << 16) | (__float_as_uint(nodes[i].costE) >> 16);
    vals[i] = i;
    return;
// ... 35 lines not shown
  const int n = min(per, B - base);
  if (n <= 0) return;
  const int t = threadIdx.x;
  const int ipt = (n + 1023) >> 10;
  const int i0 = min(n, t * ipt), i1 = min(n, i0 + ipt);
  int c = 0;
  for (int i = i0; i < i1; i++) c += S[sorder[base + i]].explore == 0;
  part[t] = c;
  __syncthreads();
  for (int d = 1; d < 1024; d <<= 1) {
    const int v = t >= d ? part[t - d] : 0;
    __syncthreads();
    part[t] += v;
    __syncthreads();
  }
  const int total = part[1023];
  int po = part[t] - c;
  int pe = i0 - po;
  for (int i = i0; i < i1; i++) {
    const int v = sorder[base + i];
    if (S[v].explore == 0) out[base + po++] = v;
    else out[base + total + pe++] = v;
  }
}

__global__ void k_walk_trun(const int* __restrict__ HEAD, const int* __restrict__ ID, int ntiles,
                            int2* __restrict__ trun) {
  const int t = blockIdx.x * blockDim.x + threadIdx.x;
  if (t >= ntiles) return;
  const int j0 = t * WALK_TILE;
  const int h = HEAD[j0];
  if (HEAD[j0 + WALK_TILE - 1] != h) {
    trun[t] = make_int2(-1, -1);
    return;
  }
  int m = 0x7fffffff;
  for (int q = 0; q < WALK_TILE; q++) m = min(m, ID[j0 + q]);
  trun[t] = m >= 0 ? make_int2(h, m) : make_int2(-1, -1);
}

__global__ void k_walk_gather(const NnRec* __restrict__ nodes, int N, int Npad, const int* __restrict__ order,
                              double ox, double oy, float4* __restrict__ P, float4* __restrict__ Q,
                              float* __restrict__ CE, int* __restrict__ ID, int* __restrict__ dup) {
  const int j = blockIdx.x * blockDim.x + threadIdx.x;
  if (j >= Npad) return;
  if (j < N) {
    const int i = order[j];
    const NnRec& r = nodes[i];
    P[j] = make_float4((float)(r.x - ox), (float)(r.y - oy), r.c, r.s);
    Q[j] = make_float4((float)(r.bx - ox), (float)(r.by - oy), r.ca, r.sa);
    CE[j] = r.costE;
    ID[j] = i;
    bool same = false;
    if (j > 0) {
      const NnRec& o = nodes[order[j - 1]];
      same = r.x == o.x && r.y == o.y && r.c == o.c && r.s == o.s && r.costE == o.costE;
    }
    dup[j] = same ? -1 : j;
  } else {
    dup[j] = j;
    P[j] = make_float4(0.f, 0.f, 1.f, 0.f);
    Q[j] = make_float4(0.f, 0.f, 1.f, 0.f);
    CE[j] = 0.f;
    ID[j] = -1;
  }
}

__device__ __forceinline__ float wsum(float v) {
#pragma unroll
  for (int o = 32; o > 0; o >>= 1) v += __shfl_xor(v, o, 64);
  return v;
}
__device__ __forceinline__ float wmax(float v) {
#pragma unroll
  for (int o = 32; o > 0; o >>= 1) v = fmaxf(v, __shfl_xor(v, o, 64));
  return v;
}
__device__ __forceinline__ float wmin(float v) {
#pragma unroll
  for (int o = 32; o > 0; o >>= 1) v = fminf(v, __shfl_xor(v, o, 64));
  return v;
}

__global__ void __launch_bounds__(256) k_walk_tiles(const float4* __restrict__ P, const float4* __restrict__ Q,
                                                    const float* __restrict__ CE, const int* __restrict__ ID,
                                                    int ntiles, int size, float slack,
                                                    const NnRec* __restrict__ nodes, double ox, double oy,
                                                    WalkTile* __restrict__ out) {
  const float Rx = (float)(nodes[0].x - ox), Ry = (float)(nodes[0].y - oy);
  const int t = blockIdx.x * (blockDim.x >> 6) + (threadIdx.x >> 6);
  const int lane = threadIdx.x & 63;
  if (t >= ntiles) return;
  const int b = t * size;
  float spx = 0, spy = 0, srx = 0, sry = 0, sux = 0, suy = 0, sax = 0, say = 0, cnt = 0, bad = 0;
  for (int k = lane; k < size; k += 64) {
    const int j = b + k;
    if (ID[j] < 0) continue;
    const float4 p = P[j], q = Q[j];
    const float ce = CE[j];
    const bool fin = isfinite(p.x) && isfinite(p.y) && isfinite(p.z) && isfinite(p.w) && isfinite(q.x) &&
                     isfinite(q.y) && isfinite(q.z) && isfinite(q.w) && isfinite(ce);
    if (!fin) { bad += 1; continue; }
    spx += p.x; spy += p.y; srx += q.x; sry += q.y;
    sux += p.z; suy -= p.w;
    sax += q.z; say += q.w;
    cnt += 1;
  }
  cnt = wsum(cnt);
  bad = wsum(bad);
  WalkTile w;
  w.nonfinite = bad > 0;
  w.eroot = 0.f;
  if (cnt == 0) {
    w.pcx = w.pcy = w.rcx = w.rcy = 0.f;
    w.pr = w.rr = -1.f;
    w.thx = 1.f; w.thy = 0.f; w.thh = 4.f;
    w.apx = 1.f; w.apy = 0.f; w.aph = 4.f;
    w.cemin = w.aopt = w.eroot = 0.f;
    if (lane == 0) out[t] = w;
    return;
  }
  const float pcx = wsum(spx) / cnt, pcy = wsum(spy) / cnt;
  const float rcx = wsum(srx) / cnt, rcy = wsum(sry) / cnt;
  float ux = wsum(sux), uy = wsum(suy), ax = wsum(sax), ay = wsum(say);
  const float un = sqrtf(ux * ux + uy * uy), an = sqrtf(ax * ax + ay * ay);
  const bool uok = un > 1e-3f * cnt, aok = an > 1e-3f * cnt;
  ux = uok ? ux / un : 1.f; uy = uok ? uy / un : 0.f;
  ax = aok ? ax / an : 1.f; ay = aok ? ay / an : 0.f;
  float pr = 0, rr = 0, ud = 1, ad = 1, cmin = __builtin_inff(), aopt = __builtin_inff(), eroot = __builtin_inff();
  for (int k = lane; k < size; k += 64) {
    const int j = b + k;
    if (ID[j] < 0) continue;
    const float4 p = P[j], q = Q[j];
    const float ce = CE[j];
    const bool fin = isfinite(p.x) && isfinite(p.y) && isfinite(p.z) && isfinite(p.w) && isfinite(q.x) &&
                     isfinite(q.y) && isfinite(q.z) && isfinite(q.w) && isfinite(ce);
    if (!fin) continue;
    const float dp = sqrtf((p.x - pcx) * (p.x - pcx) + (p.y - pcy) * (p.y - pcy));
    const float dr = sqrtf((q.x - rcx) * (q.x - rcx) + (q.y - rcy) * (q.y - rcy));
    pr = fmaxf(pr, dp);
    rr = fmaxf(rr, dr);
    const float hn = sqrtf(p.z * p.z + p.w * p.w), qn = sqrtf(q.z * q.z + q.w * q.w);
    ud = fminf(ud, (p.z * ux - p.w * uy) / hn);
    ad = fminf(ad, (q.z * ax + q.w * ay) / qn);
    cmin = fminf(cmin, ce);
    aopt = fminf(aopt, ce - dp);
    eroot = fminf(eroot, ce - sqrtf((p.x - Rx) * (p.x - Rx) + (p.y - Ry) * (p.y - Ry)));
  }
  pr = wmax(pr); rr = wmax(rr); ud = wmin(ud); ad = wmin(ad); cmin = wmin(cmin); aopt = wmin(aopt);
  eroot = wmin(eroot);
  w.pcx = pcx; w.pcy = pcy; w.pr = pr * (1.f + 1e-5f) + 2.f * slack + 1e-5f;
  w.rcx = rcx; w.rcy = rcy; w.rr = rr * (1.f + 1e-5f) + 2.f * slack + 1e-5f;
  w.thx = ux; w.thy = uy; w.thh = uok ? acosf(fminf(fmaxf(ud, -1.f), 1.f)) + 2e-3f : 4.f;
  w.apx = ax; w.apy = ay; w.aph = aok ? acosf(fminf(fmaxf(ad, -1.f), 1.f)) + 2e-3f : 4.f;
  w.cemin = cmin;
  w.aopt = aopt - 2.f * slack - 1e-4f - 1e-5f * fabsf(aopt);
  w.eroot = eroot - 2.f * slack - 1e-4f - 1e-5f * fabsf(eroot);
  if (lane == 0) out[t] = w;
}

__device__ __forceinline__ float fsqrt(float x) { return __builtin_amdgcn_sqrtf(x); }
__device__ __forceinline__ float frcp(float x) { return __builtin_amdgcn_rcpf(x); }

__device__ __forceinline__ float acos_apx(float x) {
  const float ax = fminf(fabsf(x), 1.f);
  const float r = fsqrt(1.f - ax) * (1.5707288f + ax * (-0.2121144f + ax * (0.0742610f + ax * -0.0187293f)));
  return x < 0.f ? 3.14159265f - r : r;
}

__device__ __forceinline__ float atan2_apx(float y, float x) {
  const float ax = fabsf(x), ay = fabsf(y);
  const float z = fminf(ax, ay) * frcp(fmaxf(ax, ay));
  const float z2 = z * z;
  float p = 0.0028662257f;
  p = p * z2 - 0.0161657367f;
  p = p * z2 + 0.0429096138f;
  p = p * z2 - 0.0752896400f;
  p = p * z2 + 0.1065626393f;
  p = p * z2 - 0.1420889944f;
  p = p * z2 + 0.1999355085f;
  p = p * z2 - 0.3333314528f;
  float a = z + z * z2 * p;
  if (ay > ax) a = 1.57079633f - a;
  if (x < 0.f) a = 3.14159265f - a;
  return y < 0.f ? -a : a;
}

template <bool BRK>
__device__ __forceinline__ void walk_key_range(float tx, float ty, float pos_err, float& lo, float& hi) {
  const float rho = 4.77f;
  const float t2 = tx * tx + ty * (ty - 2.f * rho);
  if (t2 <= -0.01f) {
    lo = 14.9f;
    hi = __builtin_inff();
    if constexpr (BRK) {
      const float df2 = tx * tx + (ty + rho) * (ty + rho);
      const float cA = fminf(fmaxf((5.f * rho * rho - df2) * (1.f / (4.f * rho * rho)), -1.f), 1.f);
      const float sA = fsqrt(fmaxf((1.f - cA) * (1.f + cA), 0.f));
      const float u = rho * sA;
      const float w = fsqrt(fmaxf(df2 - u * u, 0.f));
      const float cw = w * frcp(fsqrt(df2));
      if (sA >= 0.05f && cw >= 0.05f) {
        const float alpha = 6.28318531f - atan2_apx(sA, cA);
        const float L = rho * (alpha + atan2_apx(tx, ty + rho) + atan2_apx(u, w));
        const float m = 2e-3f + 1e-4f * L + pos_err * (8.f + 8.f * frcp(sA) + 8.f * frcp(cw));
        lo = fmaxf(L - m, 14.9f);
        hi = L + m;
      }
    }
    return;
  }
  if (!(t2 > -0.01f)) {
    lo = -__builtin_inff();
    hi = __builtin_inff();
    return;
  }
  const float t = fsqrt(fmaxf(t2, 0.f));
  float th = atan2_apx(tx, rho - ty);
  if (th < 0.f) th += 6.28318531f;
  const float L = t + rho * (th - atan2_apx(t, rho));
  const float m = 2.f * pos_err + 2e-4f + 2e-5f * L;
  if (t2 >= 0.01f) {
    lo = L - m;
    hi = L + m;
  } else {
    lo = fminf(L - m - 1e-4f, 14.9f);
    hi = __builtin_inff();
  }
}

__device__ __forceinline__ float walk_lb(const WalkTile& w, float rsx, float rsy, bool ex, float flen,
                                         float dsR = 0.f) {
  if (w.nonfinite) return -__builtin_inff();
  if (w.pr < 0.f) return __builtin_inff();
  const float rho = 4.77f;
  const float ex2 = rsx - w.rcx, ey2 = rsy - w.rcy;
  const float E2 = fsqrt(ex2 * ex2 + ey2 * ey2);
  if (E2 + w.rr < flen) return __builtin_inff();
  if (E2 > w.rr && w.aph < 3.f) {
    const float iE = frcp(E2);
    const float a2 = 1.57079633f - acos_apx(w.rr * iE);
    const float ang2 = acos_apx((ex2 * w.apx + ey2 * w.apy) * iE);
// ... 4 lines not shown
  float lb = D - w.pr;
  if (D > w.pr && w.thh < 3.f) {
    const float iD = frcp(D);
    const float al = 1.57079633f - acos_apx(w.pr * iD);
    const float bmin = acos_apx((dx * w.thx + dy * w.thy) * iD) - al - w.thh - 3e-3f;
    lb = fmaxf(lb, rho * bmin);
  }
  lb = lb - 2e-3f - 1e-5f * fabsf(lb);
  if (!ex) lb = fmaxf(fmaxf(w.aopt + D * (1.f - 1e-5f) - 2e-3f, w.cemin + lb), w.eroot + dsR);
  return lb == lb ? lb : -__builtin_inff();
}

#ifndef WALK_CHEAP_FIRST
#define WALK_CHEAP_FIRST 1
#endif
__device__ __forceinline__ float walk_lb_dist(const WalkTile& w, float rsx, float rsy, bool ex, float dsR = 0.f) {
  if (w.nonfinite) return -__builtin_inff();
  if (w.pr < 0.f) return __builtin_inff();
  const float dx = rsx - w.pcx, dy = rsy - w.pcy;
  const float D = fsqrt(dx * dx + dy * dy);
  float lb = D - w.pr;
  lb = lb - 2e-3f - 1e-5f * fabsf(lb);
  if (!ex) lb = fmaxf(fmaxf(w.aopt + D * (1.f - 1e-5f) - 2e-3f, w.cemin + lb), w.eroot + dsR);
  return lb == lb ? lb : -__builtin_inff();
}

__device__ __forceinline__ float uni(float v) {
  return __int_as_float(__builtin_amdgcn_readfirstlane(__float_as_int(v)));
}
__device__ __forceinline__ int uni(int v) { return __builtin_amdgcn_readfirstlane(v); }

__device__ __forceinline__ bool w_less(float ka, int ia, float kb, int ib) {
  return (ka < kb) || (ka == kb && ia < ib);
}

__device__ __forceinline__ void w_insert(float& lk, int& li, float k, int i, int lane) {
  const bool before = w_less(lk, li, k, i) && lane < NN_K;
  const int pos = __popcll(__ballot(before));
  const float uk = __shfl_up(lk, 1, 64);
  const int ui = __shfl_up(li, 1, 64);
  if (lane < NN_K) {
    if (lane == pos) { lk = k; li = i; }
    else if (lane > pos) { lk = uk; li = ui; }
  }
}

__device__ __forceinline__ void walk_emit(float lk, int li, int lane, int s, int sort_limit, int* __restrict__ cand,
                                          float* __restrict__ ckey, int* __restrict__ ncand, int* __restrict__ ctie) {
  const bool valid = lane < NN_K && li != 0x7fffffff;
  const int nvalid = __popcll(__ballot(valid));
  const int sel = min(sort_limit, nvalid);
  const float nk = __shfl_down(lk, 1, 64);
  const bool tie = lane < CAND_K && lane < sel && lane + 1 < nvalid && lk == nk;
  const bool anytie = __ballot(tie) != 0;
  if (lane < CAND_K) {
    cand[s * CAND_K + lane] = lane < sel ? li : -1;
    ckey[s * CAND_K + lane] = lk;
  }
  if (lane == 0) {
    ncand[s] = sel;
    ctie[s] = anytie;
  }
}

__device__ __forceinline__ float lc_dec(int c) {
  return c == 0 ? -__builtin_inff() : (c == 255 ? __builtin_inff() : exp2f((float)(c - 64) * 0.0625f));
}
__device__ __forceinline__ int lc_enc(float b) {
  if (b == __builtin_inff()) return 255;
  if (!(b >= lc_dec(1))) return 0;
  int c = (int)floorf(log2f(b) * 16.f) + 64;
  c = c < 1 ? 1 : (c > 254 ? 254 : c);
  while (c > 1 && lc_dec(c) > b) c--;
  while (c < 254 && lc_dec(c + 1) <= b) c++;
  return c;
}
__device__ __forceinline__ int lc_le(float v) {
  return v == __builtin_inff() ? 255 : lc_enc(v);
}

#ifndef CLRRT_WALK_WAVES
#define CLRRT_WALK_WAVES 5
#endif
template <int FMT, bool SPLIT, bool BRK>
__device__ __forceinline__ void walk_one(const clrrt_sample* __restrict__ S, int B,
                                                    const NnRec* __restrict__ nodes, const float4* __restrict__ P,
                                                    const float4* __restrict__ Q, const float* __restrict__ CE,
                                                    const int* __restrict__ ID, const int* __restrict__ HEAD,
                                                    const int2* __restrict__ trun,
                                                    const WalkTile* __restrict__ tiles, int ntiles,
                                                    const WalkTile* __restrict__ sup, int nsup, DevParams p,
                                                    NnFrame fr, int* __restrict__ cand, float* __restrict__ ckey,
                                                    int* __restrict__ ncand, int* __restrict__ ctie,
                                                    const int* __restrict__ sorder,
                                                    unsigned long long* __restrict__ stats, int bud_tiles,
                                                    int bud_ex, int* __restrict__ ovf_n, int4* __restrict__ ovf,
                                                    int max_over, int nch, float* __restrict__ pk,
                                                    int* __restrict__ pi, int nloc_max, int s, int ch, int nloc, float kb, int ib, int o_sp) {
  constexpr bool STATE = FMT == WALK_FMT_STATE, CODED = FMT == WALK_FMT_CODED;
  extern __shared__ uint8_t s_lb[];
  __half* s_lbh = (__half*)s_lb;
  __half* s_sh = s_lbh + nloc_max;
  float* s_lbf = (float*)s_lb;
  uint32_t* s_vis = (uint32_t*)(s_lbf + nloc_max);
  __shared__ int s_q2[64];
  __shared__ float s_b2[64];
#if WALK_STAGE1_QUEUE
  __shared__ int s_q1[192];
#endif
  __shared__ int s_tq[WALK_TQ];
  __shared__ float s_tb[WALK_TQ];
  const int lane = threadIdx.x;
  auto gst = [&](int l) -> int { return SPLIT ? ch + l * nch : l; };
  const double sx = S[s].x, sy = S[s].y;
  const bool ex = S[s].explore != 0;
  const float rsx = (float)(sx - fr.ox), rsy = (float)(sy - fr.oy);
  const float dl = fr.delta;
  const float flen = (float)p.feas_len - 2.f * dl;
  const float fl2 = flen > 0.f ? flen * flen : 0.f;
  const float c45 = 0.69276f;
  const float rho = 4.77f, rin = rho - 0.01f - 4.f * dl;
  const float rin2 = rin > 0.f ? rin * rin : -1.f;
  const float flen_t = (float)p.feas_len * (1.f - 1e-5f) - 4.f * dl;
  const float Rx = (float)(nodes[0].x - fr.ox), Ry = (float)(nodes[0].y - fr.oy);
  const float dsR = sqrtf((rsx - Rx) * (rsx - Rx) + (rsy - Ry) * (rsy - Ry)) * (1.f - 1e-5f) - 2.f * dl - 1e-4f;
  float lk = __builtin_inff();
  int li = 0x7fffffff;
  float uk = __builtin_inff();
  float kth = __builtin_inff();
  int kth_c = 255;
  float base = 0.f;
  int idk = 0x7fffffff;
  float lim = __builtin_inff();
  float cb0 = -2.f;
  int n2 = 0;
#ifdef CLRRT_WALK_PROFILE
  const bool prof = fr.debug == 2;
#else
  constexpr bool prof = false;
#endif
  uint64_t cyc[4] = {0, 0, 0, 0};
#ifdef CLRRT_WALK_PROFILE
  unsigned long long hist[6] = {0, 0, 0, 0, 0, 0};
#endif
  int hc = -1;
  float kc = 0.f;
  unsigned long long n_sup = 0, n_tile = 0, n_q = 0, n_ex = 0, n_und = 0, n_sure = 0, n_drop = 0;

  auto refresh = [&]() __attribute__((always_inline)) {
    kth = uni(__shfl(lk, NN_K - 1, 64));
    idk = uni(__shfl(li, NN_K - 1, 64));
    if (SPLIT && w_less(kb, ib, kth, idk)) { kth = kb; idk = ib; }
    const float u10 = uni(__shfl(uk, NN_K - 1, 64));
    if (u10 < kth) { kth = u10; idk = 0x7fffffff; }
#if WALK_SPLIT_SHARE
    if constexpr (SPLIT) {
      int* sh = &ovf[o_sp].w;
      if (lane == 0 && kth < __builtin_inff() && !(kth < 0.f)) atomicMin(sh, kth > 0.f ? __float_as_int(kth) : 0);
      const float shv = __int_as_float(uni(__atomic_load_n(sh, __ATOMIC_RELAXED)));
      if (shv < kth) { kth = shv; idk = 0x7fffffff; }
    }
#endif
    if constexpr (CODED) kth_c = uni(lc_le(kth - base));
    if (kth < __builtin_inff()) {
      const float R = (kth + 2e-4f) * (1.0f / 0.9999f);
      lim = uni(R < 0.f ? -1.f : (R + dl) * (R + dl));
      const float b0 = (kth + 0.01f) * (1.f / rho) + 2e-3f;
      cb0 = uni(b0 < 3.1f ? __cosf(b0) - 1e-4f : -2.f);
    }
  };
  auto drain_exact = [&](int room) __attribute__((always_inline)) {
    if (n2 == 0) return;
    {
      const int jj = lane < n2 ? s_q2[lane] : 0;
      const float bb = lane < n2 ? s_b2[lane] : 0.f;
      const bool k2 = lane < n2 && !(bb > kth);
      const uint64_t m2 = __ballot(k2);
      __builtin_amdgcn_wave_barrier();
      if (k2) {
        const int pos = __popcll(m2 & ((1ull << lane) - 1));
        s_q2[pos] = jj;
        s_b2[pos] = bb;
      }
      __builtin_amdgcn_wave_barrier();
      n_drop += n2 - __popcll(m2);
      n2 = __popcll(m2);
      if (n2 == 0 || n2 + room <= 64) return;
    }
    const int nq = n2;
    const uint64_t c0 = prof ? __builtin_amdgcn_s_memtime() : 0;
    n_ex += nq;
    bool c = false;
    float key = 0.f;
    int id = 0, j = 0;
    if (lane < nq) {
      j = s_q2[lane];
      id = ID[j];
      const NnRec& r = nodes[id];
      key = dubins_key(sx, sy, r.x, r.y, r.c, r.s);
      if (!ex) key = r.costE + key;
      if (w_less(key, id, kth, idk)) {
        c = feasible_search(sx, sy, r.bx, r.by, r.ca, r.sa, r.ang_par, p.feas_len);
      }
    }
    {
      const int hd = lane < nq ? HEAD[j] : 0;
      const int depth = lane < nq ? j - hd : -1;
      int best = depth;
#pragma unroll
      for (int o = 32; o > 0; o >>= 1) best = max(best, __shfl_xor(best, o, 64));
      best = uni(best);
      if (best > 0) {
        const int l = __ffsll((unsigned long long)__ballot(depth == best)) - 1;
        kc = uni(__shfl(key, l, 64));
        hc = uni(__shfl(hd, l, 64));
      }
    }
#ifdef CLRRT_WALK_PROFILE
    if (prof) {
      const float gap = key - kth;
      const bool v = lane < nq;
      hist[0] += __popcll(__ballot(v && !(gap > 0.f)));
      hist[1] += __popcll(__ballot(v && gap > 0.f && gap <= 1e-3f));
      hist[2] += __popcll(__ballot(v && gap > 1e-3f && gap <= 1e-2f));
      hist[3] += __popcll(__ballot(v && gap > 1e-2f && gap <= 0.1f));
      hist[4] += __popcll(__ballot(v && gap > 0.1f));
      hist[5] += __popcll(__ballot(v && kth == __builtin_inff()));
    }
#endif
    uint64_t m = __ballot(c);
    while (m) {
      const int l = __ffsll((unsigned long long)m) - 1;
      m &= m - 1;
      const float k = __shfl(key, l, 64);
      const int i = __shfl(id, l, 64);
      if (w_less(k, i, kth, idk)) {
        w_insert(lk, li, k, i, lane);
        refresh();
      }
// ... 97 lines not shown
    const int b0 = n1 - cnt;
    const bool v = lane < cnt;
    const int j = v ? s_q1[b0 + lane] : -1;
    __builtin_amdgcn_wave_barrier();
    n1 = b0;
    float4 pp = make_float4(0.f, 0.f, 1.f, 0.f), qq = pp;
    float ce = 0.f;
    if (v) { pp = P[j]; qq = Q[j]; ce = CE[j]; }
    float lt, ut;
    stage1(v, pp, qq, ce, lt, ut);
    n_und += __popcll(__ballot(lt == -__builtin_inff()));
    n_sure += __popcll(__ballot(ut < __builtin_inff()));
    if (ub_insert(ut)) refresh();
    enqueue(v, lt, j);
  };
#endif
  auto visit4 = [&](int t0, int t1, int t2, int t3) __attribute__((always_inline)) {
    const uint64_t c0 = prof ? __builtin_amdgcn_s_memtime() : 0;
    n_tile += (t0 >= 0) + (t1 >= 0) + (t2 >= 0) + (t3 >= 0);
    const int ta = lane < 32 ? t0 : t1, tb = lane < 32 ? t2 : t3;
    const int ja = ta >= 0 ? ta * WALK_TILE + (lane & 31) : -1;
    const int jb = tb >= 0 ? tb * WALK_TILE + (lane & 31) : -1;
    int ida = -1, idb = -1, ha = -2, hb = -2;
    float4 pa = make_float4(0.f, 0.f, 1.f, 0.f), qa = pa, pb = pa, qb = pa;
    float ca = 0.f, cb = 0.f;
    if (ja >= 0) { ida = ID[ja]; ha = HEAD[ja]; pa = P[ja]; qa = Q[ja]; ca = CE[ja]; }
    if (jb >= 0) { idb = ID[jb]; hb = HEAD[jb]; pb = P[jb]; qb = Q[jb]; cb = CE[jb]; }
    const bool oka = prefilter(ida, ha, pa, qa, ca);
    const bool okb = prefilter(idb, hb, pb, qb, cb);
    n_q += __popcll(__ballot(oka)) + __popcll(__ballot(okb));
#if WALK_STAGE1_QUEUE
    push1(oka, ja);
    push1(okb, jb);
    while (n1 >= 64) run_stage1(64);
#else
    float la, ua, lb, ub;
    stage1(oka, pa, qa, ca, la, ua);
    stage1(okb, pb, qb, cb, lb, ub);
    n_und += __popcll(__ballot(la == -__builtin_inff())) + __popcll(__ballot(lb == -__builtin_inff()));
    n_sure += __popcll(__ballot(ua < __builtin_inff())) + __popcll(__ballot(ub < __builtin_inff()));
    const bool ia = ub_insert(ua);
    const bool ib2 = ub_insert(ub);
    if (ia || ib2) refresh();
    enqueue(oka, la, ja);
    enqueue(okb, lb, jb);
#endif
    if (prof) cyc[2] += __builtin_amdgcn_s_memtime() - c0;
  };
  auto hmin = [&](float v) -> float {
#pragma unroll
    for (int o = 16; o > 0; o >>= 1) v = fminf(v, __shfl_xor(v, o, 64));
    return v;
  };
  auto run_out = [&](int tl) -> bool {
    const int2 tr = trun[tl];
    return tr.x >= 0 && tr.x == hc && !w_less(kc, tr.y, kth, idk);
  };
  int qn = 0;
  auto next_q = [&]() __attribute__((always_inline)) -> int {
    while (qn > 0) {
      qn--;
      const int t = uni(s_tq[qn]);
      if (!(uni(s_tb[qn]) > kth)) return t;
    }
    return -1;
  };
  auto visit_queue = [&]() __attribute__((always_inline)) {
    const int t0 = next_q();
    const int t1 = next_q();
    const int t2 = next_q();
    const int t3 = next_q();
    if (t0 >= 0) visit4(t0, t1, t2, t3);
    __builtin_amdgcn_wave_barrier();
  };
  auto flush_queue = [&]() __attribute__((always_inline)) {
    while (qn > 0) visit_queue();
#if WALK_STAGE1_QUEUE
    while (n1 > 0) run_stage1(n1 < 64 ? n1 : 64);
#endif
  };
  auto visit_supers = [&](int la, int lb2, float Tp, float T, bool first) {
    const uint64_t c0 = prof ? __builtin_amdgcn_s_memtime() : 0;
#if WALK_SPLIT_SHARE
    if constexpr (SPLIT) refresh();
#endif
    n_sup += 1 + (lb2 >= 0);
    const int sa = gst(la), sb = lb2 >= 0 ? gst(lb2) : -1;
    const int lo = lane < 32 ? la : lb2;
    const int st = lane < 32 ? sa : sb;
    const int tl = st * WALK_SUPER + (lane & 31);
    float lb = __builtin_inff();
    uint64_t tm;
    if constexpr (STATE) {
      const uint32_t vis = st >= 0 ? s_vis[lo] : 0xffffffffu;
      if (st >= 0 && tl < ntiles && !((vis >> (lane & 31)) & 1u)) {
#if WALK_CHEAP_FIRST
        const WalkTile tt = tiles[tl];
        lb = walk_lb_dist(tt, rsx, rsy, ex, dsR);
        if (!(lb > fminf(T, kth))) lb = walk_lb(tt, rsx, rsy, ex, flen_t, dsR);
#else
        lb = walk_lb(tiles[tl], rsx, rsy, ex, flen_t, dsR);
#endif
        if (run_out(tl)) lb = __builtin_inff();
      }
      const bool take = st >= 0 && lb <= T && !(lb > kth);
      const bool drop = st >= 0 && lb > kth;
      tm = __ballot(take);
      const uint64_t dm = __ballot(drop);
      const float rest = hmin(take || drop || st < 0 ? __builtin_inff() : lb);
      if ((lane & 31) == 0 && st >= 0) {
        const int sh = lane;
        s_vis[lo] = vis | (uint32_t)(tm >> sh) | (uint32_t)(dm >> sh);
        s_lbf[lo] = rest;
      }
    } else {
      float slb;
      if constexpr (FMT == WALK_FMT_HALF && WALK_HALF_SUPER) {
        slb = st >= 0 ? __half2float(s_sh[lo]) : __builtin_inff();
      } else {
        float sl = __builtin_inff();
        if ((lane & 31) == 0 && st >= 0) sl = walk_lb(sup[st], rsx, rsy, ex, flen_t, dsR);
        slb = __shfl(sl, lane & 32, 64);
      }
#ifdef WALK_CHEAP_STATELESS
      if (st >= 0 && tl < ntiles) {
        const WalkTile tt = tiles[tl];
        lb = fmaxf(walk_lb_dist(tt, rsx, rsy, ex, dsR), slb);
        if (!(lb > fminf(T, kth))) lb = fmaxf(walk_lb(tt, rsx, rsy, ex, flen_t, dsR), slb);
      }
#else
      if (st >= 0 && tl < ntiles) lb = fmaxf(walk_lb(tiles[tl], rsx, rsy, ex, flen_t, dsR), slb);
#endif
      if (st >= 0 && tl < ntiles && run_out(tl)) lb = __builtin_inff();
      const bool take = st >= 0 && (first || lb > Tp) && lb <= T && !(lb > kth);
      tm = __ballot(take);
      const float rest = hmin(st >= 0 && lb > T ? lb : __builtin_inff());
      if ((lane & 31) == 0 && st >= 0) {
        if constexpr (CODED) s_lb[lo] = (uint8_t)lc_enc(rest - base);
        else s_lbh[lo] = __float2half_rd(rest);
      }
    }
    const bool tk = (tm >> lane) & 1ull;
    if (tk) {
      const int pos = qn + __popcll(tm & ((1ull << lane) - 1));
      s_tq[pos] = st * WALK_SUPER + (lane & 31);
      s_tb[pos] = lb;
    }
    qn += __popcll(tm);
    __builtin_amdgcn_wave_barrier();
    while (qn >= 4) visit_queue();
    if (prof) cyc[1] += __builtin_amdgcn_s_memtime() - c0;
  };

  const uint64_t ct0 = prof ? __builtin_amdgcn_s_memtime() : 0;
  auto flush_stats = [&]() {
    if (stats && lane == 0) {
      atomicAdd(&stats[0], n_sup);
      atomicAdd(&stats[1], n_tile);
      atomicAdd(&stats[2], n_q);
      atomicAdd(&stats[3], n_ex);
      atomicAdd(&stats[10], n_und);
      atomicAdd(&stats[11], n_sure);
      atomicAdd(&stats[12], n_drop);
      if (prof) {
        atomicAdd(&stats[4], (unsigned long long)cyc[0]);
        atomicAdd(&stats[5], (unsigned long long)cyc[1]);
        atomicAdd(&stats[6], (unsigned long long)cyc[2]);
        atomicAdd(&stats[7], (unsigned long long)cyc[3]);
        atomicAdd(&stats[8], (unsigned long long)(__builtin_amdgcn_s_memtime() - ct0));
#ifdef CLRRT_WALK_PROFILE
        atomicAdd(&stats[13], hist[0]);
        for (int q = 1; q < 6; q++) atomicAdd(&stats[14 + q], hist[q]);
#endif
      }
    }
  };
  if (SPLIT) refresh();
  float mlb = __builtin_inff();
  for (int t0 = 0; t0 < nloc; t0 += 64) {
    const int t = t0 + lane;
    if (t < nloc) {
      const float lb = walk_lb(sup[gst(t)], rsx, rsy, ex, flen_t, dsR);
      if constexpr (STATE) {
        s_lbf[t] = lb;
        s_vis[t] = 0u;
      } else if constexpr (!CODED) {
        s_lbh[t] = __float2half_rd(lb);
        if constexpr (WALK_HALF_SUPER) s_sh[t] = s_lbh[t];
      }
      mlb = fminf(mlb, lb);
    }
  }
  mlb = wmin(mlb);
  base = mlb > 0.f && mlb < __builtin_inff() ? mlb : 0.f;
  if constexpr (CODED) {
    for (int t0 = 0; t0 < nloc; t0 += 64) {
      const int t = t0 + lane;
      if (t < nloc) s_lb[t] = (uint8_t)lc_enc(walk_lb(sup[gst(t)], rsx, rsy, ex, flen_t, dsR) - base);
    }
  }
  __builtin_amdgcn_wave_barrier();
  if (prof) cyc[0] += __builtin_amdgcn_s_memtime() - ct0;
#ifndef WALK_T0
#define WALK_T0 0.5f
#endif
#ifndef WALK_GROW
#define WALK_GROW 2.f
#endif
  float T = base + WALK_T0, Tp = -__builtin_inff();
  bool budget = !SPLIT && (bud_tiles > 0 || bud_ex > 0);
  for (int pass = 0;; pass++) {
    const float lim_t = fminf(T, kth);
    const int lim_c = CODED ? uni(lc_le(lim_t - base)) : 0;
    for (int t0 = 0; t0 < nloc; t0 += 64) {
      const int t = t0 + lane;
      bool want;
      if constexpr (CODED) {
        const int c = t < nloc ? s_lb[t] : 255;
        want = c != 255 && c <= lim_c;
      } else {
        const float lb = t < nloc ? (STATE ? s_lbf[t] : __half2float(s_lbh[t])) : __builtin_inff();
        want = lb < __builtin_inff() && lb <= lim_t;
      }
      uint64_t m = __ballot(want);
      while (m) {
        int sa = -1, sb = -1;
        while (m && sb < 0) {
          const int st = t0 + __ffsll((unsigned long long)m) - 1;
          m &= m - 1;
          if (CODED ? (int)s_lb[st] > kth_c : (STATE ? s_lbf[st] : __half2float(s_lbh[st])) > kth) continue;
          if (sa < 0) sa = st; else sb = st;
        }
        if (sa >= 0) visit_supers(sa, sb, Tp, T, pass == 0);
        if (budget && ((bud_tiles > 0 && n_tile > (unsigned long long)bud_tiles) ||
                       (bud_ex > 0 && n_ex > (unsigned long long)bud_ex))) {
          int slot = 0;
          if (lane == 0) slot = atomicAdd(ovf_n, 1);
          slot = uni(__shfl(slot, 0, 64));
          if (slot < max_over) {
            if (lane == 0)
              ovf[slot] = make_int4(s, __float_as_int(kth), idk == 0x7fffffff ? idk : idk + 1,
                                    kth > 0.f ? __float_as_int(kth) : kth == 0.f ? 0 : 0x7f800000);
            if (stats && lane == 0) atomicAdd(&stats[14], 1ull);
            flush_stats();
            return;
          }
          budget = false;
        }
      }
    }
    flush_queue();
    drain();
    if (T == __builtin_inff() || kth <= T) break;
    Tp = T;
    T = base + (T - base) * WALK_GROW;
    if (T > 1e7f) T = __builtin_inff();
  }
  if constexpr (SPLIT) {
    const int o = o_sp;
    if (lane < NN_K) {
      pk[((size_t)o * nch + ch) * NN_K + lane] = lk;
      pi[((size_t)o * nch + ch) * NN_K + lane] = li;
    }
  } else {
    walk_emit(lk, li, lane, s, p.sort_limit, cand, ckey, ncand, ctie);
  }
  flush_stats();
}

template <int FMT, bool SPLIT, bool BRK, bool PERS = false>
__global__ void __launch_bounds__(64) __attribute__((amdgpu_waves_per_eu(CLRRT_WALK_WAVES))) k_walk_search(const clrrt_sample* __restrict__ S, int B,
                                                    const NnRec* __restrict__ nodes, const float4* __restrict__ P,
                                                    const float4* __restrict__ Q, const float* __restrict__ CE,
                                                    const int* __restrict__ ID, const int* __restrict__ HEAD,
                                                    const int2* __restrict__ trun,
                                                    const WalkTile* __restrict__ tiles, int ntiles,
                                                    const WalkTile* __restrict__ sup, int nsup, DevParams p,
                                                    NnFrame fr, int* __restrict__ cand, float* __restrict__ ckey,
                                                    int* __restrict__ ncand, int* __restrict__ ctie,
                                                    const int* __restrict__ sorder,
                                                    unsigned long long* __restrict__ stats, int bud_tiles,
                                                    int bud_ex, int* __restrict__ ovf_n, int4* __restrict__ ovf,
                                                    int max_over, int nch, float* __restrict__ pk,
                                                    int* __restrict__ pi, int nloc_max, int* __restrict__ wctr) {
  if constexpr (SPLIT) {
    const int o = (int)blockIdx.x / nch;
    const int ch = (int)blockIdx.x % nch;
    if (o >= min(*ovf_n, max_over)) return;
    const int4 rec = ovf[o];
    const int nloc = ch < nsup ? (nsup - ch + nch - 1) / nch : 0;
    walk_one<FMT, SPLIT, BRK>(S, B, nodes, P, Q, CE, ID, HEAD, trun, tiles, ntiles, sup, nsup, p, fr, cand, ckey, ncand, ctie, sorder, stats, bud_tiles, bud_ex, ovf_n, ovf, max_over, nch, pk, pi, nloc_max, rec.x, ch, nloc, __int_as_float(rec.y), rec.z, o);
  } else {
// ... 409 lines not shown
                                       : fmt == WALK_FMT_HALF ? (WALK_HALF_SUPER ? 2 : 1) * sizeof(__half)
                                                              : 1) *
                                          (size_t)nsup);
  const bool pers_k = w.waves > 0 && w.wctr && B >= w.waves_min_batch;
  const void* kfn =
      fmt == WALK_FMT_STATE ? (pers_k ? (const void*)&k_walk_search<WALK_FMT_STATE, false, false, true>
                                      : (const void*)&k_walk_search<WALK_FMT_STATE, false, false, false>)
      : fmt == WALK_FMT_HALF ? (pers_k ? (const void*)&k_walk_search<WALK_FMT_HALF, false, false, true>
                                       : (const void*)&k_walk_search<WALK_FMT_HALF, false, false, false>)
                             : (pers_k ? (const void*)&k_walk_search<WALK_FMT_CODED, false, true, true>
                                       : (const void*)&k_walk_search<WALK_FMT_CODED, false, true, false>);
  if (lds > 64 * 1024) {
    e = hipFuncSetAttribute(kfn, hipFuncAttributeMaxDynamicSharedMemorySize, (int)lds);
    if (e != hipSuccess) return e;
  }
  const bool split = (w.bud_tiles > 0 || w.bud_ex > 0) && w.max_over > 0 && w.nch > 0 && w.ovf_n;
  const bool pers_z = w.waves > 0 && w.wctr && B >= w.waves_min_batch;
  hipLaunchKernelGGL(k_walk_skeys, dim3((B + 255) / 256), dim3(256), 0, st, S, B, x0, y0, scale, w.keys, w.vals,
                     split ? w.ovf_n : nullptr, pers_z ? w.wctr : nullptr);
  LAUNCH_CHECK3();
  bytes = w.tmp_bytes;
  e = hipcub::DeviceRadixSort::SortPairs(w.tmp, bytes, w.keys, w.keys2, w.vals, w.sorder, B, 0, 32, st);
  if (e != hipSuccess) return e;
  const int* sorder = w.sorder;
  if (w.lpt && B >= 8) {
    hipLaunchKernelGGL(k_walk_lpt, dim3(8), dim3(1024), 0, st, S, B, (const int*)w.sorder, (int*)w.keys2);
    LAUNCH_CHECK3();
    sorder = (const int*)w.keys2;
  }
  const int bt = split ? w.bud_tiles : 0, be = split ? w.bud_ex : 0;
  const bool pers = pers_k;
  const int grid = pers ? std::min(((B + 7) >> 3) * 8, std::max(8, w.waves & ~7)) : ((B + 7) >> 3) * 8;
  int* wctr = pers ? w.wctr : nullptr;
#define WALK_LAUNCH1(F, BK, PS)                                                                                  \
  hipLaunchKernelGGL((k_walk_search<F, false, BK, PS>), dim3(grid), dim3(64), lds, st, S, B, nodes, w.P,          \
                     w.Q, w.CE, w.ID, w.HEAD, w.trun, w.tiles, ntiles, w.supers, nsup, p, fr, cand, ckey, ncand, ctie,  \
                     sorder, stats, bt, be, w.ovf_n, w.ovf, w.max_over, w.nch, w.pk, w.pi, nsup, wctr)
#define WALK_LAUNCH(F, BK)            \
  do {                                \
    if (pers) WALK_LAUNCH1(F, BK, true);  \
    else WALK_LAUNCH1(F, BK, false);  \
  } while (0)
  if (fmt == WALK_FMT_STATE) WALK_LAUNCH(WALK_FMT_STATE, false);
  else if (fmt == WALK_FMT_HALF) WALK_LAUNCH(WALK_FMT_HALF, false);
  else WALK_LAUNCH(WALK_FMT_CODED, true);
#undef WALK_LAUNCH
#undef WALK_LAUNCH1
  LAUNCH_CHECK3();
  if (w.seed_out) {
    hipLaunchKernelGGL(k_walk_seed, dim3((B + 63) / 64), dim3(64), 0, st, B, p.sort_limit, (const float*)ckey,
                       (const int*)ncand, w.seed_out);
    LAUNCH_CHECK3();
    if (split) {
      hipLaunchKernelGGL(k_walk_seed_ovf, dim3((w.max_over + 63) / 64), dim3(64), 0, st, (const int*)w.ovf_n,
                         (const int4*)w.ovf, w.max_over, w.seed_out);
      LAUNCH_CHECK3();
    }
  }
  if (w.ev_main && (e = hipEventRecord(w.ev_main, st)) != hipSuccess) return e;
  if (split) {
    const int nl = (nsup + w.nch - 1) / w.nch;
    const void* sfn = brk ? (const void*)&k_walk_search<WALK_FMT_STATE, true, true>
                          : (const void*)&k_walk_search<WALK_FMT_STATE, true, false>;
    if (2 * sizeof(float) * (size_t)nl > 64 * 1024) {
      e = hipFuncSetAttribute(sfn, hipFuncAttributeMaxDynamicSharedMemorySize, (int)(2 * sizeof(float) * (size_t)nl));
      if (e != hipSuccess) return e;
    }
#define WALK_SPLIT(BK)                                                                                           \
  hipLaunchKernelGGL((k_walk_search<WALK_FMT_STATE, true, BK>), dim3(w.max_over * w.nch), dim3(64),               \
                     2 * sizeof(float) * (size_t)nl, st, S, B, nodes, w.P, w.Q, w.CE, w.ID, w.HEAD, w.trun, w.tiles, \
                     ntiles, w.supers, nsup, p, fr, cand, ckey, ncand, ctie, sorder, stats, 0, 0, w.ovf_n, w.ovf,  \
                     w.max_over, w.nch, w.pk, w.pi, nl, nullptr)
    if (brk) WALK_SPLIT(true);
    else WALK_SPLIT(false);
#undef WALK_SPLIT
    LAUNCH_CHECK3();
    hipLaunchKernelGGL(k_walk_merge, dim3(w.max_over), dim3(64), 0, st, w.ovf_n, w.ovf, w.max_over, w.nch, w.pk, w.pi,
                       p.sort_limit, cand, ckey, ncand, ctie);
    LAUNCH_CHECK3();
  }
  return hipSuccess;
}

}
```

Measured before the change: 1.333 million.

## Replace brute-force delta NN scan with a spatial walk index over new nodes

For the lagged nearest-neighbour delta step (nodes added since a sample's tree snapshot), the code now builds a small sorted tile/super-tile walk index over just the delta nodes, using key generation, a radix sort and a fused range-index kernel. It then runs a pruned walk search per sample instead of the brute-force chunked partial scan. The old split-delta path and its buffers are removed, and an optional verify mode compares results against brute force. The aim is to cut the O(B×delta) distance work, at the cost of extra sort and index-build launches per round, which may dominate when the delta is small.

```diff
diff --git a/cl-rrt_amd/csrc/clrrt_capi.hip b/cl-rrt_amd/csrc/clrrt_capi.hip
--- a/cl-rrt_amd/csrc/clrrt_capi.hip
+++ b/cl-rrt_amd/csrc/clrrt_capi.hip
@@ -166,17 +166,17 @@
   WalkBufs nnw3{};
   hipStream_t side2 = nullptr;
   hipStream_t mst = nullptr;
-  int nn_split_delta = 0;
+  int nn_delta_walk = 1;
+  int nn_delta_verify = 0;
+  WalkBufs nnw_d{};
+  float* vpk = nullptr;
+  int* vpi = nullptr;
+  float* vseed = nullptr;
   int nn_delta_early = 1;
   int nn_lane_order = 1;
   int* nn_order = nullptr;
   float* wseed[3] = {nullptr, nullptr, nullptr};
   hipEvent_t ev_wm[3] = {nullptr, nullptr, nullptr};
-  float* nn_seed2 = nullptr;
-  float* d1pk[3] = {nullptr, nullptr, nullptr};
-  int* d1pi[3] = {nullptr, nullptr, nullptr};
-  hipEvent_t ev_d1[3] = {nullptr, nullptr, nullptr};
-  hipEvent_t ev_s[3] = {nullptr, nullptr, nullptr};
   hipEvent_t ev_lagw[3] = {nullptr, nullptr, nullptr};
   int stream_prio = 1;
   int walk_cu_reserve = 0;
@@ -503,15 +503,17 @@
   if (c->mst) hipStreamSynchronize(c->mst);
   if (c->mst) hipStreamDestroy(c->mst);
   for (int q = 0; q < 3; q++) {
-    if (c->ev_d1[q]) hipEventDestroy(c->ev_d1[q]);
-    if (c->ev_s[q]) hipEventDestroy(c->ev_s[q]);
-    if (c->d1pk[q]) hipFree(c->d1pk[q]);
     if (c->wseed[q]) hipFree(c->wseed[q]);
     if (q == 0 && c->nn_order) hipFree(c->nn_order);
     if (c->ev_wm[q]) hipEventDestroy(c->ev_wm[q]);
-    if (c->d1pi[q]) hipFree(c->d1pi[q]);
-  }
-  if (c->nn_seed2) hipFree(c->nn_seed2);
+  }
+  {
+    WalkBufs& d = c->nnw_d;
+    void* wd[] = {d.keys, d.vals, d.tmp, d.P, d.Q, d.CE, d.ID, d.HEAD, d.trun, d.tiles, d.supers, d.skeys, d.sids,
+                  c->vpk, c->vpi, c->vseed};
+    for (void* p : wd)
+      if (p) hipFree(p);
+  }
   if (c->side) hipStreamSynchronize(c->side);
   if (c->ev_tree) hipEventDestroy(c->ev_tree);
   if (c->ev_walk) hipEventDestroy(c->ev_walk);
@@ -1280,7 +1282,8 @@
   }
   else if (k == "nn_walk_double") c->nnw_double = value != 0;
   else if (k == "nn_lag" && (value == 0 || value == 1 || value == 2)) c->nn_lag = (int)value;
-  else if (k == "nn_split_delta") c->nn_split_delta = value != 0 ? 1 : 0;
+  else if (k == "nn_delta_walk") c->nn_delta_walk = value != 0 ? 1 : 0;
+  else if (k == "nn_delta_verify") c->nn_delta_verify = value != 0 ? 1 : 0;
   else if (k == "nn_delta_early") c->nn_delta_early = value != 0 ? 1 : 0;
   else if (k == "nn_lane_order") c->nn_lane_order = value != 0 ? 1 : 0;
   else if (k == "nn_debug" && value >= 0) c->nn_debug = (int)value;
@@ -2443,12 +2446,6 @@
   int64_t g = 0;
   int64_t tree_n = 0;
   int stream = 0;
-  float* d1pk = nullptr;
-  int* d1pi = nullptr;
-  int d1_chunks = 0;
-  int64_t d1_count = 0;
-  hipEvent_t evd1 = nullptr;
-  hipEvent_t evs = nullptr;
   float* wseed = nullptr;
   hipEvent_t evm = nullptr;
 };
@@ -2474,15 +2471,43 @@
     HIPC(c, hipStreamCreateWithFlags(&c->side2, hipStreamNonBlocking));
   }
   HIPC(c, hipStreamCreateWithFlags(&c->mst, hipStreamNonBlocking));
-  HIPC(c, dalloc(&c->nn_seed2, B));
   for (int q = 0; q < 3; q++) {
-    HIPC(c, dalloc(&c->d1pk[q], c->partial_cap));
     HIPC(c, dalloc(&c->wseed[q], B));
     if (q == 0) HIPC(c, dalloc(&c->nn_order, B));
     HIPC(c, hipEventCreateWithFlags(&c->ev_wm[q], hipEventDisableTiming));
-    HIPC(c, dalloc(&c->d1pi[q], c->partial_cap));
-    HIPC(c, hipEventCreateWithFlags(&c->ev_d1[q], hipEventDisableTiming));
-    HIPC(c, hipEventCreateWithFlags(&c->ev_s[q], hipEventDisableTiming));
+  }
+  return CLRRT_OK;
+}
+
+static int alloc_walk_delta(clrrt_ctx* c) {
+  WalkBufs& w = c->nnw_d;
+  if (!w.P) {
+    const int64_t cap = walk_delta_cap(c->cap.max_nodes, c->cap.max_batch);
+    const int64_t Mp = walk_tile_count(cap) * 32;
+    HIPC(c, dalloc(&w.keys, 2 * cap));
+    HIPC(c, dalloc(&w.vals, cap));
+    w.tmp_bytes = walk_sort_bytes((int)cap);
+    HIPC(c, hipMalloc(&w.tmp, std::max<size_t>(w.tmp_bytes, 256)));
+    HIPC(c, dalloc(&w.skeys, cap));
+    HIPC(c, dalloc(&w.sids, cap));
+    HIPC(c, dalloc(&w.Q, Mp));
+    HIPC(c, dalloc(&w.CE, Mp));
+    HIPC(c, dalloc(&w.ID, Mp));
+    HIPC(c, dalloc(&w.HEAD, Mp));
+    HIPC(c, dalloc(&w.trun, walk_tile_count(cap)));
+    HIPC(c, dalloc(&w.tiles, walk_tile_count(cap)));
+    HIPC(c, dalloc(&w.supers, walk_super_count(cap)));
+    w.sorted_n = -1;
+    w.cap_nodes = cap;
+    w.cap_batch = (int)c->cap.max_batch;
+    HIPC(c, dalloc(&w.P, Mp));
+  }
+  w.index_kind = c->nnw_index;
+  w.hscale_pct = c->nnw_hscale;
+  if (c->nn_delta_verify && !c->vseed) {
+    HIPC(c, dalloc(&c->vpk, c->partial_cap));
+    HIPC(c, dalloc(&c->vpi, c->partial_cap));
+    HIPC(c, dalloc(&c->vseed, c->cap.max_batch));
   }
   return CLRRT_OK;
 }
@@ -2522,6 +2547,7 @@
 static int expand_lag2(clrrt_ctx* c, clrrt_rng* rng, int64_t n_iters, double budget_ms, int32_t batch,
                        clrrt_stats* out) {
   int rc = lag_alloc(c);
+  if (rc == CLRRT_OK && c->nn_delta_walk) rc = alloc_walk_delta(c);
   if (rc == CLRRT_OK) rc = apply_stream_prio(c);
   if (rc == CLRRT_OK) rc = defer_begin(c, true);
   if (rc != CLRRT_OK) return rc;
@@ -2546,8 +2572,6 @@
   A.ctie = c->ctie2; A.ev = c->ev_lag[0]; A.evw = c->ev_lagw[0];
   B.d = c->d_samples3; B.h = c->h_samples3; B.cand = c->cand3; B.ckey = c->ckey3; B.ncand = c->ncand3;
   B.ctie = c->ctie3; B.ev = c->ev_lag[1]; B.evw = c->ev_lagw[1];
-  A.d1pk = c->d1pk[0]; A.d1pi = c->d1pi[0]; A.evd1 = c->ev_d1[0]; A.evs = c->ev_s[0];
-  B.d1pk = c->d1pk[1]; B.d1pi = c->d1pi[1]; B.evd1 = c->ev_d1[1]; B.evs = c->ev_s[1];
   A.wseed = c->wseed[0]; A.evm = c->ev_wm[0];
   B.wseed = c->wseed[1]; B.evm = c->ev_wm[1];
   float* cur_wseed = c->wseed[2];
@@ -2555,10 +2579,8 @@
   const bool early = c->nn_delta_early != 0;
   hipEvent_t cur_ev = c->ev_lag[2];
   hipEvent_t cur_evw = c->ev_lagw[2];
-  float* cur_d1pk = c->d1pk[2];
-  int* cur_d1pi = c->d1pi[2];
-  hipEvent_t cur_evd1 = c->ev_d1[2], cur_evs = c->ev_s[2];
-  const bool split_delta = c->nn_split_delta != 0;
+  const int64_t delta_walk_min = 32;
+  const bool delta_walk = c->nn_delta_walk != 0;
   struct RoleGuard {
     std::function<void()> f;
     ~RoleGuard() { f(); }
@@ -2603,9 +2625,6 @@
     c->nn_samples += n;
     HIPC(c, hipStreamWaitEvent(s, c->ev_tree, 0));
     HIPC(c, hipMemcpyAsync(sl.d, sl.h, sizeof(clrrt_sample) * n, hipMemcpyHostToDevice, s));
-    HIPC(c, hipEventRecord(sl.evs, s));
-    sl.d1_count = 0;
-    sl.d1_chunks = 0;
     c->nn_super_bounds += (int64_t)n * walk_super_count(c->n_nodes);
     {
       KTimer kt(c, 0, s), kt3(c, 3, s);
@@ -2713,87 +2732,50 @@
     if ((rc = compact_and_copy(c, L, &nn, true)) != CLRRT_OK) break;
     const double ms_commit = std::chrono::duration<double, std::milli>(std::chrono::steady_clock::now() - t0).count();
     if ((rc = commit_round(c, nn, ms_commit, &n_app)) != CLRRT_OK) break;
-    if ((A.n > 0 || (split_delta && B.n > 0)))
+    if (A.n > 0) {
       HIPC(c, hipEventRecord(c->ev_commit, c->stream));
-    if (A.n > 0 && split_delta) {
       hipStream_t s = c->mst;
       HIPC(c, hipStreamWaitEvent(s, c->ev_commit, 0));
       HIPC(c, hipStreamWaitEvent(s, early ? A.evm : A.evw, 0));
-      const int64_t first2 = A.tree_n + A.d1_count, cnt2 = c->n_nodes - first2;
-      int nch2 = 0;
-      if (cnt2 > 0) {
+      const int64_t first = A.tree_n, cnt = c->n_nodes - A.tree_n;
+      const NnSetup su2 = nn_setup(c);
+      const bool dwalk = delta_walk && su2.region_ok && c->n_nodes >= c->nnw_min_nodes && cnt >= delta_walk_min &&
+                         cnt <= c->nnw_d.cap_nodes;
+      const int max_chunks = (int)std::max<int64_t>(1, c->partial_cap / ((int64_t)A.n * NN_K));
+      int nch = 0, id0 = (int)first;
+      if (cnt > 0) c->nn_bf_keys += (int64_t)A.n * cnt;
+      if (cnt > 0 && dwalk) {
         KTimer kt(c, 0, s);
-        c->nn_bf_keys += (int64_t)A.n * cnt2;
-        const NnSetup su2 = nn_setup(c);
-        const int max_chunks = (int)std::max<int64_t>(1, c->partial_cap / ((int64_t)A.n * NN_K));
-        HIPC(c, launch_nn_delta_partial(s, A.d, A.n, c->nn, (int)first2, (int)cnt2, c->dp, su2.fr, c->pk, c->pi,
-                                        max_chunks, A.ckey, A.ncand, early ? A.wseed : c->nn_seed, early,
-                                        c->nn_lane_order ? c->nn_order : nullptr, &nch2));
-      }
-      if (early) HIPC(c, hipStreamWaitEvent(s, A.evw, 0));
-      if (A.d1_count > 0) HIPC(c, hipStreamWaitEvent(s, A.evd1, 0));
-      {
+        float* seed = early ? A.wseed : c->nn_seed;
+        const bool verify = c->nn_delta_verify && c->vseed;
+        HIPC(c, launch_nn_delta_walk(s, A.d, A.n, c->nn, (int)first, (int)cnt, c->dp, su2.fr, su2.x0, su2.y0, su2.x1,
+                                     su2.y1, c->nnw_d, c->pk, c->pi, A.ckey, A.ncand, seed, early,
+                                     verify ? c->work_ctr + 40 : nullptr));
+        nch = 1;
+        id0 = 0;
+        if (verify) {
+          int vch = 0;
+          HIPC(c, hipMemcpyAsync(c->vseed, seed, sizeof(float) * A.n, hipMemcpyDeviceToDevice, s));
+          HIPC(c, launch_nn_delta_partial(s, A.d, A.n, c->nn, (int)first, (int)cnt, c->dp, su2.fr, c->vpk, c->vpi,
+                                          max_chunks, nullptr, nullptr, c->vseed, true, nullptr, &vch, c->work_ctr + 52));
+          HIPC(c, launch_nn_delta_compare(s, A.n, vch, (int)first, c->vpk, c->vpi, c->pk, c->pi, c->work_ctr + 38));
+        }
+      } else if (cnt > 0 && early) {
         KTimer kt(c, 0, s);
-        if (A.d1_count > 0)
-          HIPC(c, launch_nn_delta_merge(s, A.n, A.d1_chunks, c->dp, A.d1pk, A.d1pi, (int)A.tree_n, A.cand, A.ckey,
-                                        A.ncand, A.ctie));
-        HIPC(c, launch_nn_delta_merge(s, A.n, nch2, c->dp, c->pk, c->pi, (int)first2, A.cand, A.ckey, A.ncand, A.ctie));
-      }
-      HIPC(c, hipEventRecord(A.ev, s));
-    } else if (A.n > 0 && early) {
-      hipStream_t s = c->mst;
-      HIPC(c, hipStreamWaitEvent(s, c->ev_commit, 0));
-      HIPC(c, hipStreamWaitEvent(s, A.evm, 0));
-      const int64_t first = A.tree_n, cnt = c->n_nodes - A.tree_n;
-      int nch = 0;
-      if (cnt > 0) {
-        KTimer kt(c, 0, s);
-        c->nn_bf_keys += (int64_t)A.n * cnt;
-        const NnSetup su2 = nn_setup(c);
-        const int max_chunks = (int)std::max<int64_t>(1, c->partial_cap / ((int64_t)A.n * NN_K));
         HIPC(c, launch_nn_delta_partial(s, A.d, A.n, c->nn, (int)first, (int)cnt, c->dp, su2.fr, c->pk, c->pi,
                                         max_chunks, nullptr, nullptr, A.wseed, true,
                                         c->nn_lane_order ? c->nn_order : nullptr, &nch));
-      }
-      HIPC(c, hipStreamWaitEvent(s, A.evw, 0));
-      {
+      } else if (cnt > 0) {
         KTimer kt(c, 0, s);
-        HIPC(c, launch_nn_delta_merge(s, A.n, nch, c->dp, c->pk, c->pi, (int)first, A.cand, A.ckey, A.ncand, A.ctie));
-      }
-      HIPC(c, hipEventRecord(A.ev, s));
-    } else if (A.n > 0) {
-      hipStream_t s = c->mst;
-      HIPC(c, hipStreamWaitEvent(s, c->ev_commit, 0));
-      HIPC(c, hipStreamWaitEvent(s, A.evw, 0));
-      const int64_t first = A.tree_n, cnt = c->n_nodes - A.tree_n;
-      if (cnt > 0) {
-        KTimer kt(c, 0, s);
-        c->nn_bf_keys += (int64_t)A.n * cnt;
-        const NnSetup su2 = nn_setup(c);
-        const int max_chunks = (int)std::max<int64_t>(1, c->partial_cap / ((int64_t)A.n * NN_K));
         HIPC(c, launch_nn_delta(s, A.d, A.n, c->nn, (int)first, (int)cnt, c->dp, su2.fr, c->pk, c->pi, max_chunks,
                                 A.cand, A.ckey, A.ncand, A.ctie, c->nn_seed));
       }
+      if (early) HIPC(c, hipStreamWaitEvent(s, A.evw, 0));
+      if (nch > 0) {
+        KTimer kt(c, 0, s);
+        HIPC(c, launch_nn_delta_merge(s, A.n, nch, c->dp, c->pk, c->pi, id0, A.cand, A.ckey, A.ncand, A.ctie));
+      }
       HIPC(c, hipEventRecord(A.ev, s));
-    }
-    if (split_delta && B.n > 0) {
-      hipStream_t s2 = c->mst;
-      HIPC(c, hipStreamWaitEvent(s2, c->ev_commit, 0));
-      HIPC(c, hipStreamWaitEvent(s2, B.evs, 0));
-      HIPC(c, hipStreamWaitEvent(s2, early ? B.evm : B.evw, 0));
-      const int64_t cnt1 = c->n_nodes - B.tree_n;
-      B.d1_count = cnt1;
-      B.d1_chunks = 0;
-      if (cnt1 > 0) {
-        KTimer kt(c, 0, s2);
-        c->nn_bf_keys += (int64_t)B.n * cnt1;
-        const NnSetup su1 = nn_setup(c);
-        const int max_chunks = (int)std::max<int64_t>(1, c->partial_cap / ((int64_t)B.n * NN_K));
-        HIPC(c, launch_nn_delta_partial(s2, B.d, B.n, c->nn, (int)B.tree_n, (int)cnt1, c->dp, su1.fr, B.d1pk, B.d1pi,
-                                        max_chunks, B.ckey, B.ncand, early ? B.wseed : c->nn_seed2, early,
-                                        c->nn_lane_order ? c->nn_order : nullptr, &B.d1_chunks));
-      }
-      HIPC(c, hipEventRecord(B.evd1, s2));
     }
     {
       const NnSetup sn = nn_setup(c);
@@ -2812,14 +2794,12 @@
       LagSlot old;
       old.d = c->d_samples; old.h = c->h_samples; old.cand = c->cand; old.ckey = c->ckey; old.ncand = c->ncand;
       old.ctie = c->ctie; old.ev = cur_ev; old.evw = cur_evw; old.stream = cur_stream;
-      old.d1pk = cur_d1pk; old.d1pi = cur_d1pi; old.evd1 = cur_evd1; old.evs = cur_evs;
       old.wseed = cur_wseed; old.evm = cur_evm;
       have_cur = A.n > 0;
       c->d_samples = A.d; c->h_samples = A.h; c->cand = A.cand; c->ckey = A.ckey; c->ncand = A.ncand; c->ctie = A.ctie;
       cur_ev = A.ev;
       cur_evw = A.evw;
       cur_stream = A.stream;
-      cur_d1pk = A.d1pk; cur_d1pi = A.d1pi; cur_evd1 = A.evd1; cur_evs = A.evs;
       cur_wseed = A.wseed; cur_evm = A.evm;
       A = B;
       B = old;
diff --git a/cl-rrt_amd/csrc/clrrt_internal.hpp b/cl-rrt_amd/csrc/clrrt_internal.hpp
--- a/cl-rrt_amd/csrc/clrrt_internal.hpp
+++ b/cl-rrt_amd/csrc/clrrt_internal.hpp
@@ -193,10 +193,17 @@
 hipError_t launch_nn_delta(hipStream_t st, const clrrt_sample* S, int B, const NnRec* nodes, int first, int count,
                            const DevParams& p, const NnFrame& fr, float* pk, int* pi, int max_chunks, int* cand,
                            float* ckey, int* ncand, int* ctie, float* seed);
+int64_t walk_delta_cap(int64_t max_nodes, int64_t max_batch);
+hipError_t launch_nn_delta_walk(hipStream_t st, const clrrt_sample* S, int B, const NnRec* nodes, int first, int count,
+                                const DevParams& p, const NnFrame& fr, double x0, double y0, double x1, double y1,
+                                WalkBufs& w, float* pk, int* pi, const float* ckey, const int* ncand, float* seed,
+                                bool seeded, unsigned long long* stats);
+hipError_t launch_nn_delta_compare(hipStream_t st, int B, int nchunks, int id0, const float* pk, const int* pi,
+                                   const float* wk, const int* wi, unsigned long long* out);
 hipError_t launch_nn_delta_partial(hipStream_t st, const clrrt_sample* S, int B, const NnRec* nodes, int first,
                                    int count, const DevParams& p, const NnFrame& fr, float* pk, int* pi, int max_chunks,
                                    const float* ckey, const int* ncand, float* gcap, bool seeded, int* order,
-                                   int* nchunks_out);
+                                   int* nchunks_out, unsigned long long* tstat = nullptr);
 hipError_t launch_nn_delta_merge(hipStream_t st, int B, int nchunks, const DevParams& p, const float* pk, const int* pi,
                                  int id0, int* cand, float* ckey, int* ncand, int* ctie);
 hipError_t launch_nn(hipStream_t st, const clrrt_sample* S, int B, const NnRec* nodes, int N,
diff --git a/cl-rrt_amd/csrc/clrrt_kernels.hip b/cl-rrt_amd/csrc/clrrt_kernels.hip
--- a/cl-rrt_amd/csrc/clrrt_kernels.hip
+++ b/cl-rrt_amd/csrc/clrrt_kernels.hip
@@ -309,6 +309,33 @@
   }
   ncand[s] = n;
   ctie[s] = tie;
+}
+
+__global__ void k_nn_delta_compare(int B, int nchunks, int id0, const float* __restrict__ pk,
+                                   const int* __restrict__ pi, const float* __restrict__ wk,
+                                   const int* __restrict__ wi, unsigned long long* __restrict__ out) {
+  const int s = blockIdx.x * blockDim.x + threadIdx.x;
+  if (s >= B) return;
+  float keys[NN_K];
+  int ids[NN_K];
+#pragma unroll
+  for (int j = 0; j < NN_K; j++) { keys[j] = __builtin_inff(); ids[j] = 0x7fffffff; }
+  for (int c = 0; c < nchunks; c++) {
+    const size_t base = ((size_t)s * nchunks + c) * NN_K;
+    for (int j = 0; j < NN_K; j++) {
+      const int id = pi[base + j];
+      if (id == 0x7fffffff) break;
+      const float k = pk[base + j];
+      if (lex_less(k, id + id0, keys[NN_K - 1], ids[NN_K - 1])) topk_insert(keys, ids, k, id + id0);
+      else break;
+    }
+  }
+  bool bad = false;
+#pragma unroll
+  for (int j = 0; j < NN_K; j++)
+    bad |= __float_as_uint(keys[j]) != __float_as_uint(wk[(size_t)s * NN_K + j]) || ids[j] != wi[(size_t)s * NN_K + j];
+  atomicAdd(&out[0], 1ull);
+  if (bad) atomicAdd(&out[1], 1ull);
 }
 
 __global__ void k_nn_exact(const clrrt_sample* __restrict__ S, int B, const NnRec* __restrict__ nodes, int N,
@@ -2537,7 +2564,7 @@
 hipError_t launch_nn_delta_partial(hipStream_t st, const clrrt_sample* S, int B, const NnRec* nodes, int first,
                                    int count, const DevParams& p, const NnFrame& fr, float* pk, int* pi, int max_chunks,
                                    const float* ckey, const int* ncand, float* gcap, bool seeded, int* order,
-                                   int* nchunks_out) {
+                                   int* nchunks_out, unsigned long long* tstat) {
   *nchunks_out = 0;
   if (count <= 0 || B <= 0) return hipSuccess;
   const int* sord = nullptr;
@@ -2559,7 +2586,7 @@
     LAUNCH_CHECK();
   }
   hipLaunchKernelGGL(k_nn_partial, dim3(groups, nchunks), dim3(CLRRT_PATH_BLK), 0, st, S, B, nodes + first, count, chunk,
-                     nchunks, p, fr, pk, pi, gcap, nullptr, sord);
+                     nchunks, p, fr, pk, pi, gcap, tstat, sord);
   LAUNCH_CHECK();
   *nchunks_out = nchunks;
   return hipSuccess;
@@ -2569,6 +2596,14 @@
   if (nchunks <= 0 || B <= 0) return hipSuccess;
   hipLaunchKernelGGL(k_nn_merge_delta, dim3((B + 63) / 64), dim3(64), 0, st, B, nchunks, p.sort_limit, pk, pi, id0, cand,
                      ckey, ncand, ctie);
+  LAUNCH_CHECK();
+  return hipSuccess;
+}
+
+hipError_t launch_nn_delta_compare(hipStream_t st, int B, int nchunks, int id0, const float* pk, const int* pi,
+                                   const float* wk, const int* wi, unsigned long long* out) {
+  if (B <= 0) return hipSuccess;
+  hipLaunchKernelGGL(k_nn_delta_compare, dim3((B + 63) / 64), dim3(64), 0, st, B, nchunks, id0, pk, pi, wk, wi, out);
   LAUNCH_CHECK();
   return hipSuccess;
 }
diff --git a/cl-rrt_amd/csrc/clrrt_nnwalk.hip b/cl-rrt_amd/csrc/clrrt_nnwalk.hip
--- a/cl-rrt_amd/csrc/clrrt_nnwalk.hip
+++ b/cl-rrt_amd/csrc/clrrt_nnwalk.hip
@@ -27,6 +27,9 @@
 #define WALK_TQ 68
 #ifndef WALK_SPLIT_SHARE
 #define WALK_SPLIT_SHARE 1
+#endif
+#ifndef CLRRT_DELTA_ONEPASS
+#define CLRRT_DELTA_ONEPASS 1
 #endif
 #ifndef WALK_APBINS
 #define WALK_APBINS 8
@@ -228,15 +231,8 @@
   return v;
 }
 
-__global__ void __launch_bounds__(256) k_walk_tiles(const float4* __restrict__ P, const float4* __restrict__ Q,
-                                                    const float* __restrict__ CE, const int* __restrict__ ID,
-                                                    int ntiles, int size, float slack,
-                                                    const NnRec* __restrict__ nodes, double ox, double oy,
-                                                    WalkTile* __restrict__ out) {
-  const float Rx = (float)(nodes[0].x - ox), Ry = (float)(nodes[0].y - oy);
-  const int t = blockIdx.x * (blockDim.x >> 6) + (threadIdx.x >> 6);
-  const int lane = threadIdx.x & 63;
-  if (t >= ntiles) return;
+__device__ __forceinline__ void walk_tile_bounds(const float4* P, const float4* Q, const float* CE, const int* ID, int t,
+                                                 int size, float slack, float Rx, float Ry, int lane, WalkTile* out) {
   const int b = t * size;
   float spx = 0, spy = 0, srx = 0, sry = 0, sux = 0, suy = 0, sax = 0, say = 0, cnt = 0, bad = 0;
   for (int k = lane; k < size; k += 64) {
@@ -304,6 +300,73 @@
   w.eroot = eroot - 2.f * slack - 1e-4f - 1e-5f * fabsf(eroot);
   if (lane == 0) out[t] = w;
 }
+__global__ void __launch_bounds__(256) k_walk_tiles(const float4* __restrict__ P, const float4* __restrict__ Q,
+                                                    const float* __restrict__ CE, const int* __restrict__ ID,
+                                                    int ntiles, int size, float slack,
+                                                    const NnRec* __restrict__ nodes, double ox, double oy,
+                                                    WalkTile* __restrict__ out) {
+  const float Rx = (float)(nodes[0].x - ox), Ry = (float)(nodes[0].y - oy);
+  const int t = blockIdx.x * (blockDim.x >> 6) + (threadIdx.x >> 6);
+  const int lane = threadIdx.x & 63;
+  if (t >= ntiles) return;
+  walk_tile_bounds(P, Q, CE, ID, t, size, slack, Rx, Ry, lane, out);
+}
+
+__global__ void __launch_bounds__(1024) k_walk_range_index(const NnRec* __restrict__ nodes, int n, const int* __restrict__ order,
+                                                           double ox, double oy, float slack, float4* P, float4* Q,
+                                                           float* CE, int* ID, int* HEAD, int2* trun,
+                                                           WalkTile* tiles, WalkTile* supers) {
+  __shared__ int s_h[WALK_TILE * WALK_SUPER];
+  __shared__ int s_id[WALK_TILE * WALK_SUPER];
+  const int t = threadIdx.x;
+  const int b = blockIdx.x;
+  const int j = b * (WALK_TILE * WALK_SUPER) + t;
+  int id = -1, mark = j;
+  float4 pp = make_float4(0.f, 0.f, 1.f, 0.f), qq = pp;
+  float ce = 0.f;
+  if (j < n) {
+    id = order[j];
+    const NnRec& r = nodes[id];
+    pp = make_float4((float)(r.x - ox), (float)(r.y - oy), r.c, r.s);
+    qq = make_float4((float)(r.bx - ox), (float)(r.by - oy), r.ca, r.sa);
+    ce = r.costE;
+    if (t > 0) {
+      const NnRec& o = nodes[order[j - 1]];
+      if (r.x == o.x && r.y == o.y && r.c == o.c && r.s == o.s && r.costE == o.costE) mark = -1;
+    }
+  }
+  P[j] = pp;
+  Q[j] = qq;
+  CE[j] = ce;
+  ID[j] = id;
+  s_h[t] = mark;
+  s_id[t] = id;
+  __syncthreads();
+  for (int d = 1; d < WALK_TILE * WALK_SUPER; d <<= 1) {
+    const int v = t >= d ? s_h[t - d] : -1;
+    __syncthreads();
+    s_h[t] = max(s_h[t], v);
+    __syncthreads();
+  }
+  HEAD[j] = s_h[t];
+  if (t < WALK_SUPER) {
+    const int q0 = t * WALK_TILE;
+    const int h = s_h[q0];
+    int2 tr = make_int2(-1, -1);
+    if (s_h[q0 + WALK_TILE - 1] == h) {
+      int m = 0x7fffffff;
+      for (int q = 0; q < WALK_TILE; q++) m = min(m, s_id[q0 + q]);
+      if (m >= 0) tr = make_int2(h, m);
+    }
+    trun[b * WALK_SUPER + t] = tr;
+  }
+  __syncthreads();
+  const float Rx = (float)(nodes[0].x - ox), Ry = (float)(nodes[0].y - oy);
+  const int wv = t >> 6, lane = t & 63;
+  for (int q = wv; q < WALK_SUPER; q += (WALK_TILE * WALK_SUPER) >> 6)
+    walk_tile_bounds(P, Q, CE, ID, b * WALK_SUPER + q, WALK_TILE, slack, Rx, Ry, lane, tiles);
+  if (wv == 0) walk_tile_bounds(P, Q, CE, ID, b, WALK_TILE * WALK_SUPER, slack, Rx, Ry, lane, supers);
+}
 
 __device__ __forceinline__ float fsqrt(float x) { return __builtin_amdgcn_sqrtf(x); }
 __device__ __forceinline__ float frcp(float x) { return __builtin_amdgcn_rcpf(x); }
@@ -474,7 +537,7 @@
 #ifndef CLRRT_WALK_WAVES
 #define CLRRT_WALK_WAVES 5
 #endif
-template <int FMT, bool SPLIT, bool BRK>
+template <int FMT, bool SPLIT, bool BRK, bool SHARE = SPLIT>
 __device__ __forceinline__ void walk_one(const clrrt_sample* __restrict__ S, int B,
                                                     const NnRec* __restrict__ nodes, const float4* __restrict__ P,
                                                     const float4* __restrict__ Q, const float* __restrict__ CE,
@@ -546,7 +609,7 @@
     const float u10 = uni(__shfl(uk, NN_K - 1, 64));
     if (u10 < kth) { kth = u10; idk = 0x7fffffff; }
 #if WALK_SPLIT_SHARE
-    if constexpr (SPLIT) {
+    if constexpr (SPLIT && SHARE) {
       int* sh = &ovf[o_sp].w;
       if (lane == 0 && kth < __builtin_inff() && !(kth < 0.f)) atomicMin(sh, kth > 0.f ? __float_as_int(kth) : 0);
       const float shv = __int_as_float(uni(__atomic_load_n(sh, __ATOMIC_RELAXED)));
@@ -810,7 +873,7 @@
   auto visit_supers = [&](int la, int lb2, float Tp, float T, bool first) {
     const uint64_t c0 = prof ? __builtin_amdgcn_s_memtime() : 0;
 #if WALK_SPLIT_SHARE
-    if constexpr (SPLIT) refresh();
+    if constexpr (SPLIT && SHARE) refresh();
 #endif
     n_sup += 1 + (lb2 >= 0);
     const int sa = gst(la), sb = lb2 >= 0 ? gst(lb2) : -1;
@@ -936,6 +999,11 @@
 #define WALK_GROW 2.f
 #endif
   float T = base + WALK_T0, Tp = -__builtin_inff();
+#if CLRRT_DELTA_ONEPASS
+  if constexpr (SPLIT && !SHARE) {
+    if (kb < __builtin_inff()) T = __builtin_inff();
+  }
+#endif
   bool budget = !SPLIT && (bud_tiles > 0 || bud_ex > 0);
   for (int pass = 0;; pass++) {
     const float lim_t = fminf(T, kth);
@@ -1511,4 +1579,60 @@
   return hipSuccess;
 }
 
-}
+__device__ __forceinline__ float w_dec32(unsigned int u) {
+  return __uint_as_float((u & 0x80000000u) ? (u & 0x7fffffffu) : ~u);
+}
+#ifndef CLRRT_DELTA_WAVES
+#define CLRRT_DELTA_WAVES 4
+#endif
+__global__ void __launch_bounds__(64) __attribute__((amdgpu_waves_per_eu(CLRRT_DELTA_WAVES)))
+k_walk_delta(const clrrt_sample* __restrict__ S, int B, const NnRec* __restrict__ nodes, const float4* __restrict__ P,
+             const float4* __restrict__ Q, const float* __restrict__ CE, const int* __restrict__ ID,
+             const int* __restrict__ HEAD, const int2* __restrict__ trun, const WalkTile* __restrict__ tiles, int ntiles,
+             const WalkTile* __restrict__ sup, int nsup, DevParams p, NnFrame fr, const float* __restrict__ seed,
+             unsigned long long* __restrict__ stats, float* __restrict__ pk, int* __restrict__ pi) {
+  const int s = blockIdx.x;
+  if (s >= B) return;
+  const float cap = w_dec32(((const unsigned int*)seed)[s]);
+  walk_one<WALK_FMT_STATE, true, false, false>(S, B, nodes, P, Q, CE, ID, HEAD, trun, tiles, ntiles, sup, nsup, p, fr,
+                                               nullptr, nullptr, nullptr, nullptr, nullptr, stats, 0, 0, nullptr, nullptr,
+                                               0, 1, pk, pi, nsup, s, 0, nsup, cap, 0x7fffffff, s);
+}
+
+int64_t walk_delta_cap(int64_t max_nodes, int64_t max_batch) {
+  return std::min<int64_t>(max_nodes, 6 * max_batch + 1024);
+}
+
+hipError_t launch_nn_delta_walk(hipStream_t st, const clrrt_sample* S, int B, const NnRec* nodes, int first, int count,
+                                const DevParams& p, const NnFrame& fr, double x0, double y0, double x1, double y1,
+                                WalkBufs& w, float* pk, int* pi, const float* ckey, const int* ncand, float* seed,
+                                bool seeded, unsigned long long* stats) {
+  if (count <= 0 || B <= 0) return hipSuccess;
+  if (count > w.cap_nodes) return hipErrorInvalidValue;
+  const int Npad = (count + WALK_TILE * WALK_SUPER - 1) / (WALK_TILE * WALK_SUPER) * (WALK_TILE * WALK_SUPER);
+  const int ntiles = Npad / WALK_TILE, nsup = ntiles / WALK_SUPER;
+  const int kind = w.index_kind;
+  const double hrho = 4.77 * (w.hscale_pct > 0 ? w.hscale_pct : 100) * 0.01;
+  const double span = kind ? fmax(fmax(x1 - x0, y1 - y0), 2.0 * M_PI * hrho) : fmax(x1 - x0, y1 - y0);
+  const double scale = span > 0 ? 65535.0 / span : 1.0;
+  hipLaunchKernelGGL(k_walk_keys, dim3((count + 63) / 64), dim3(64), 0, st, nodes, first + count, x0, y0, scale,
+                     (uint64_t*)w.keys, w.vals, first, kind, hrho);
+  LAUNCH_CHECK3();
+  size_t bytes = w.tmp_bytes;
+  hipError_t e = hipcub::DeviceRadixSort::SortPairs(w.tmp, bytes, (const uint64_t*)w.keys, w.skeys, w.vals, w.sids,
+                                                    count, 0, 64, st);
+  if (e != hipSuccess) return e;
+  hipLaunchKernelGGL(k_walk_range_index, dim3(nsup), dim3(WALK_TILE * WALK_SUPER), 0, st, nodes, count,
+                     (const int*)w.sids, fr.ox, fr.oy, fr.delta, w.P, w.Q, w.CE, w.ID, w.HEAD, w.trun, w.tiles, w.supers);
+  LAUNCH_CHECK3();
+  if (!seeded) {
+    hipLaunchKernelGGL(k_walk_seed, dim3((B + 63) / 64), dim3(64), 0, st, B, p.sort_limit, ckey, ncand, seed);
+    LAUNCH_CHECK3();
+  }
+  hipLaunchKernelGGL(k_walk_delta, dim3(B), dim3(64), 2 * sizeof(float) * (size_t)nsup, st, S, B, nodes, w.P, w.Q, w.CE,
+                     w.ID, w.HEAD, w.trun, w.tiles, ntiles, w.supers, nsup, p, fr, (const float*)seed, stats, pk, pi);
+  LAUNCH_CHECK3();
+  return hipSuccess;
+}
+
+}
```

After: 1.375 million (median of 6 runs). 1.03x the previous value.
